# Xi-yuanWang/GLASS

Hardware: AMD Instinct MI355X
Metric: aggregated edges/sec (GLASSConv fwd+bwd) (higher is better)
Workload: dtype f32; 1 GPU; ppi_bp-shaped synthetic graph (BASELINE config[1]): N=17080, nnz=633902, hidden=64, layers=2, aggr=mean, pool=sum, z_ratio=0.95, dropout=0.5, batch=80x10 per rank, use_deg features, Adam; parallelism=subgraph-batch dp1, replicated graph, bucketed gradient all-reduce per step, step=MaxZOZ+fwd+loss+bwd+allreduce+Adam, hip_graph=True, caller=step: bench.py calls glass_amd.step.TrainStep on pre-selected batches, labels_in_head_launch=True

## Files before the change

### glass_amd/_lib.py

```python
import ctypes
import os

import torch
from ctypes import c_void_p, c_int, c_int64, c_uint64, c_float, c_double, c_char_p, POINTER

_HERE = os.path.dirname(os.path.abspath(__file__))
LIB_PATH = os.environ.get("GLASS_HIP_LIB") or os.path.join(_HERE, "libglass_hip.so")

POOL_MODES = {"sum": 0, "mean": 1, "max": 2, "size": 3}
AGGR_MODES = {"mean": 0, "sum": 1, "gcn": 2}
SEG_MODES = {"gcn": 0, "gin": 1}
ACT_NONE, ACT_ELU, ACT_RELU = 0, 1, 2
PLAN_HEADER_WORDS = 16
EMBED_NORM_MAX_ROWS = 8192
ABI_VERSION = 6


class GlassHipError(RuntimeError):
    pass


_P = c_void_p
_I = c_int64

# ... 2 lines not shown
    _fields_ = [("acc", c_void_p), ("n_rep", c_int64), ("dy", c_void_p), ("lddy", c_int64), ("x", c_void_p), ("ldx", c_int64),
                ("addend", c_void_p), ("ldadd", c_int64), ("saved", c_void_p), ("gamma", c_void_p), ("alpha", c_void_p),
                ("dgamma", c_void_p), ("dbeta", c_void_p), ("dalpha", c_void_p), ("accumulate", c_int), ("act", c_int),
                ("p_drop", c_float), ("call_id", c_uint64)]

    @property
    def ptr(self):
        return ctypes.addressof(self)


class GnSrc(ctypes.Structure):
    _fields_ = [("acc", c_void_p), ("n_src", c_int64), ("n_rep", c_int64), ("gamma", c_void_p), ("beta", c_void_p),
                ("alpha", c_void_p), ("eps", c_float)]

    @classmethod
    def of(cls, acc, n_src, n_rep, gn):
        return cls(acc.data_ptr(), n_src, n_rep, gn.weight.data_ptr(), gn.bias.data_ptr(), gn.mean_scale.data_ptr(),
                   float(gn.eps))

    @property
    def ptr(self):
        return ctypes.addressof(self)
SIGNATURES = {
    "glass_version": (c_int, []),
    "glass_last_error_string": (c_char_p, []),
    "glass_spmm_plan_build": (c_int, [_P, _I, _P, POINTER(c_int64)]),
    "glass_spmm_ws_bytes": (c_int64, [_P, _I]),
    "glass_spmm_csr_f32": (c_int, [_P, _P, _P, _P, _I, _P, _I, _I, _I, _P, _P, _P, _P]),
    "glass_adj_values_f32": (c_int, [_P, _P, _P, _I, c_int, _P, _P, _P]),
    "glass_maxzoz_i64": (c_int, [_P, _I, _P, _I, _P]),
    "glass_embed_label_f32": (c_int, [_P, _P, _I, _P, _P, _I, _P, _I, _P, _I, _I, _P]),
    "glass_mix_fwd_f32": (c_int, [_P, _I, _P, c_double, c_int, _P, _I, _I, _I, _P]),
    "glass_mix_bwd_f32": (c_int, [_P, _I, _P, _I, _P, c_double, c_int, _P, _I, _I, _I, _P]),
    "glass_graphnorm_ws_bytes": (c_int64, [_I, _I]),
    "glass_graphnorm_fwd_f32": (c_int, [_P, _I, _P, _I, _I, _I, _P, _P, _P, c_float, _P, c_int, c_float, _P, c_uint64,
                                        _P, _P]),
    "glass_graphnorm_bwd_f32": (c_int, [_P, _I, _P, _I, _P, _I, _P, _I, _I, _I, _P, _P, _P, _P, _P, _P, c_int, c_int, c_float,
                                        _P, c_uint64, _P, _P]),
    "glass_rng_advance": (c_int, [_P, _P]),
    "glass_empty_launch": (c_int, [_I, _I, _I, _I, _I, _P]),
    "glass_dropout_scales_f32": (c_int, [_P, c_uint64, c_float, _I, _I, _P, _P]),
    "glass_dual_linear_stat_rows": (c_int64, [_I]),
    "glass_copy_pair": (c_int, [_P, _P, _I, _P, _P, _I, _P]),
    "glass_graphnorm_stats_f32": (c_int, [_P, _I, _I, _I, _P, _P, _P, c_float, _P, _P, _P]),
    "glass_readout_supported": (c_int, [_I, _I, c_int]),
    "glass_readout_ws_bytes": (c_int64, [_I, _I, _I]),
    "glass_readout_train_f32": (c_int, [_P, _I, _P, _P, _P, _P, _I, _I, c_int, _P, _P, _P, c_int, _I, _P, _P, _P, _P, _P, _I,
                                        _P, _P, c_int, _P, _P, _P, c_int, _P, _I, _I, _P, _P, _P, _P, _P, c_int, _P, _P, _P]),
    "glass_readout_scatter_ws_bytes": (c_int64, [_I, _I, _I]),
    "glass_linear_wgrad_reduce_batch_f32": (c_int, [_I, _P, _P, _P, _P, _P, _P, _P, _P, _P, _P]),
    "glass_wgrad_reduce_spmm_f32": (c_int, [_I, _P, _P, _P, _P, _P, _P, _P, _P, _P, _P, _P, _P, _P, _I, _P, _I, _I, _I, _P, _P,
                                            _P, _P]),
    "glass_spmm_reduce_rows_f32": (c_int, [_P, _P, _I, _I, _P, _I, _P]),
    "glass_segment_pool_f32": (c_int, [_P, _I, _P, _I, _I, c_int, _P, _I, _P, _I, _I, _P]),
    "glass_segment_pool_bwd_f32": (c_int, [_P, _I, _P, _I, _I, c_int, _P, _P, _I, _I, _I, _P]),
    "glass_segment_pool_bwd_atomic_f32": (c_int, [_P, _I, _P, _I, _I, c_int, _P, _P, _I, _I, _I, _P]),
    "glass_segment_pool_max_bwd_exact_f32": (c_int, [_P, _I, _P, _I, _I, _P, _P, _I, _I, _I, _P, _P]),
    "glass_pair_pool_ws_bytes": (c_int64, [_I, _I]),
    "glass_segment_pool_bwd_exact_ws_bytes": (c_int64, [_I, _I, _I]),
    "glass_segment_pool_bwd_exact_f32": (c_int, [_P, _I, _P, _I, _I, c_int, _P, _I, _I, _I, _P, _P]),
    "glass_pair_pool_f32": (c_int, [_P, _I, _P, _I, c_int, _P, _I, _I, _I, _P]),
    "glass_pair_pool_bwd_f32": (c_int, [_P, _I, _P, _I, c_int, _P, _I, _I, _I, _P, _P]),
    "glass_dense_caps_query": (c_int, [_I, _P]),
    "glass_pair_head_supported": (c_int, [_I]),
    "glass_pair_head_ws_bytes": (c_int64, [_I, _I]),
    "glass_pair_head_fwd_f32": (c_int, [_P, _I, _I, _P, _I, _P, _P, _P, _P, _P, c_float, _P, c_uint64, _P, _P, _P, _P, _P, _P]),
    "glass_pair_head_bwd_f32": (c_int, [_P, _I, _I, _P, _I, _P, _P, _P, _P, c_float, _P, _P, _P, _P, c_int, _P, _P, _I, _P, _P]),
    "glass_linear_wgrad_ws_bytes": (c_int64, [_I, _I, _I]),
    "glass_linear_wgrad_f32": (c_int, [_P, _I, _P, _I, _I, _I, _I, _P, _I, _P, c_int, _P, _P]),
    "glass_dual_linear_supported": (c_int, [_I]),
    "glass_dual_linear_layout": (c_int, [_I]),
    "glass_dual_linear_fwd_f32": (c_int, [_P, _I, _P, _I, _P, _P, _P, c_double, c_int, _P, _I, _P, _I, _I, _I, _P, c_int, _P, _P,
                                          c_int, c_float, _P, c_uint64, _P, _I, _P, _I, _P]),
    "glass_dual_linear_fwd_gather_supported": (c_int, [_I]),
    "glass_step_prologue_f32": (c_int, [_P, _P, _P, _P, _P, _P, _P, _I, _P, _P, _I, _P, _P, _P, _P, c_float, _P, _P, _I, _P, _I, _P]),
    "glass_peer_allreduce_adam_f32": (c_int, [_P, _I, _P, _P, _P, _P, c_double, c_double, c_double, c_double, _P, _P, _P, _I, _P, _P]),
    "glass_peer_alloc": (c_int, [_I, _P]),
    "glass_peer_free": (c_int, [_P]),
    "glass_peer_export": (c_int, [_P, _P]),
    "glass_peer_import": (c_int, [_P, _P]),
    "glass_peer_close": (c_int, [_P]),
    "glass_step_head_f32": (c_int, [_P, _P, _P, _P, _P, _P, _P, _I, _P, _P, _I, _P, _P, _P, _P, c_float, _P, _P, _I, _P, _I,
                                    _P, _I, _I, _I, _P, _P, _P, _P, _P, _P, _I, _P]),
    "glass_graphnorm_finalize_f32": (c_int, [_P, _I, _I, _I, _I, _P, _P, _P, c_float, _P, _P]),
    "glass_graphnorm_apply_f32": (c_int, [_P, _I, _P, _I, _I, _I, _P, c_int, c_float, _P, c_uint64, _P]),
    "glass_dual_linear_dgrad_f32": (c_int, [_P, _I, _P, _I, _P, c_double, c_int, _P, _I, _P, _I, c_float, _P, c_uint64, _P, _I,
                                            _I, _I, _P, _P, _I, _P, _P, c_int, c_float, c_uint64, c_int, _P]),
    "glass_dual_linear_bwd_f32": (c_int, [_P, _I, _P, _I, _P, c_double, c_int, _P, _I, _P, _I, c_float, _P, c_uint64, _P, _I,
                                          _I, _I, _P, _P, _I, _P, _P, c_int, c_float, c_uint64, c_int, _P, _I, _P, _I, _P, _P]),
    "glass_gn_exact_supported": (c_int, [_I]),
    "glass_gn_exact_fwd_supported": (c_int, [_I]),
    "glass_gn_exact_words": (c_int64, [_I]),
    "glass_graphnorm_stats_exact_f32": (c_int, [_P, _I, _I, _I, _P, c_int, _P]),
    "glass_graphnorm_bwd_from_stats_f32": (c_int, [_P, _I, _P, _I, _P, _I, _P, _I, _I, _I, _P, _P, _P, _P, _I, _P, _P, _P,
                                                   c_int, c_int, c_float, _P, c_uint64, _P, _P]),
    "glass_embed_norm_fwd_f32": (c_int, [_P, _P, _I, _P, _P, _P, _P, c_float, _P, _P, _P, _P, _I, c_float, _P, c_uint64, _P,
                                         _I, _P, _I, _I, _P]),
    "glass_embed_norm_bwd_f32": (c_int, [_P, _P, _I, _P, _P, _P, _P, _P, c_int, _P, _P, _P, c_int, _I, _P]),
    "glass_embed_norm_bwd_adam_f32": (c_int, [_P, _P, _I, _P, _P, _P, _P, _P, c_int, _P, _P, _P, c_int, _I, _P, _P, _I, _P, _P, _P,
                                              _P, _I, _P, c_double, c_double, c_double, c_double, _P, _I, _I, _I, _I, _P]),
    "glass_dual_linear_wgrad_f32": (c_int, [_P, _I, _P, _I, _P, c_double, c_int, _P, _I, _P, _I, _I, _I, _P, _I, _P,
                                            c_int, _P, _P]),
    "glass_dense_pack_batch_f32": (c_int, [_P, _P, _P, _P, _P, _P, _P, _I, _P, _P]),
    "glass_dense_image_floats": (_I, [_I, _I, c_int]),
    "glass_dual_linear_dgrad_layout": (c_int, [_I, _I]),
    "glass_dual_linear_fwd_layout": (c_int, [_I, _I]),
    "glass_head_loss_fwd_f32": (c_int, [_P, _I, _P, _P, _P, c_int, _I, _I, _I, _P, _P, _P, _P]),
    "glass_head_linear_f32": (c_int, [_P, _I, _P, _P, _I, _I, _I, _P, _I, _P]),
    "glass_head_loss_bwd_f32": (c_int, [_P, _I, _P, _P, _P, c_int, _P, _I, _I, _I, _P, _I, _P, _P, c_int, _P]),
    "glass_batch_labels_ws_bytes": (c_int64, [_I]),
    "glass_batch_labels": (c_int, [_P, _I, _P, _P, _P, _I, _P, _P, _P, _P, _I, c_int, _P]),
    "glass_batch_labels_gather": (c_int, [_P, _I, _I, _P, _I, _P, _I, _P, _P, _P, _P, _P, _P, _I, c_int, _P]),
    "glass_comb_eff_supported": (c_int, [_I]),
    "glass_comb_eff_blocks": (c_int64, [_I, _I, _I]),
    "glass_comb_eff_fwd_blocks": (c_int64, [_I, _I, _I]),
    "glass_comb_eff_ws_bytes": (c_int64, [_I, _I, _I]),
    "glass_comb_eff_fwd_layout": (c_int, [_I]),
    "glass_comb_eff_fwd_supported": (c_int, [_I]),
    "glass_comb_eff_max_rows": (c_int64, [_I]),
    "glass_comb_eff_dgrad_layout2": (c_int, [_I]),
    "glass_comb_eff_fwd_f32": (c_int, [_P, _I, _P, _I, _P, _P, _P, c_double, _P, _I, _I, _I, _P, c_int, _P, _P, c_int, c_float, _P,
                                       c_uint64, _P, _I, _P, _P, _I, _P]),
    "glass_comb_eff_bwd_f32": (c_int, [_P, _I, _P, c_double, _P, _P, _I, _I, _I, _P, _P, _I, _P, _P, c_int, c_float, _P,
                                       c_uint64, c_int, _P, _I, _P, _I, _P, _P, _P, _I, _P, _P]),
    "glass_comb_eff_bwd_gn_src_supported": (c_int, [_I, _I]),
    "glass_adam_step_f32": (c_int, [_P, _P, _P, _P, _I, _P, c_double, c_double, c_double, c_double, _P, _P]),
    "glass_seg_extract_count": (c_int, [_P, _P, _P, _P, _P, _I, _P, _P, _I, _I, c_int, _P, _P, _P, _P]),
    "glass_seg_extract_fill": (c_int, [_P, _P, _P, _P, _P, _P, _I, _P, _P, _I, _I, c_int, _P, _P, _P, _P, _P, _P, _P, _P]),
    "glass_seg_collate": (c_int, [_P, _P, _I, _P, _P, _P, _P, _P, _P, _P, _I, _P, _I, _P, _P, _P, _P, _P, _P, _P, _P, _I,
                                  _P]),
    "glass_seg_khop_ws_bytes": (c_int64, [_I, _I]),
    "glass_seg_khop_count": (c_int, [_P, _P, _I, _P, _P, _I, _I, c_int, _P, _I, _P, _P]),
    "glass_seg_khop_fill": (c_int, [_P, _P, _I, _P, _P, _I, _I, c_int, _P, _I, _P, _P, _P]),
}

_lib = None


class DenseCaps(ctypes.Structure):
    _fields_ = [(n, ctypes.c_int32) for n in ("family", "weight_layout", "fwd_layout_trans", "fwd_layout_comb", "dgrad_layout_trans",
                                              "dgrad_layout_comb", "stat_rows", "fwd_gather", "gn_exact", "gn_exact_fwd", "comb_eff",
                                              "comb_eff_fwd", "comb_eff_fwd_layout", "comb_eff_dgrad_layout2", "pair_head", "act_codes",
                                              "product_form", "serve_width")]


_caps = {}


def dense_caps(H):
    c = _caps.get(int(H))
    if c is None:
        c = DenseCaps()
        check(load().glass_dense_caps_query(int(H), ctypes.addressof(c)), "glass_dense_caps_query")
        _caps[int(H)] = c
    return c


ACT_MASK = 0xff
DENSE_F32_PRODUCTS = 0x100


def load():
    global _lib
    if _lib is not None:
        return _lib
    if not os.path.exists(LIB_PATH):
# ... 19 lines not shown
```

### glass_amd/arena.py

```python
import torch

from .dist import FlatGradBucket


def _pairs(model):
    from .models import GLASSConv, MyGCNConv
    out = []
    for m in model.modules():
        if isinstance(m, GLASSConv):
            out.append((m, "trans", m.trans_fns[1], m.trans_fns[0]))
            out.append((m, "comb", m.comb_fns[1], m.comb_fns[0]))
        elif isinstance(m, MyGCNConv):
            out.append((m, "trans", None, m.trans_fn))
            out.append((m, "comb", None, m.comb_fn))
    return out


BIG_PARAM_ELEMS = 1 << 18

_RUNTIME_ATTRS = ("_glass_grad_bucket", "_glass_arena", "_glass_stack_prog", "_stack", "_stack_eff", "_direct_grad", "_sel_cache",
                  "_chan_cache", "_glass_train_steps", "_glass_eval_graphs", "_glass_adopted_adam")


def drop_captured_graphs(model):
# ... 83 lines not shown
            self.big_start = total
        self._exchange = None
        self.shard_optimizer = False
        self.model = model
        model._glass_grad_bucket = self
        self.params = params
        self.flat_param = torch.zeros(total, dtype=dtype, device=dev)
        self.flat = torch.zeros(total, dtype=dtype, device=dev)
        self._offsets = offsets
        drop_captured_graphs(model)
        with torch.no_grad():
            for p in params:
                o = offsets[id(p)]
                view = self.flat_param[o:o + p.numel()].view_as(p)
                view.copy_(p.data)
                p.data = view
                p.grad = self.flat[o:o + p.numel()].view_as(p)
        from .models import MyGCNConv
        for mod in model.modules():
            if isinstance(mod, (GLASSConv, MyGCNConv)):
                mod._stack = {}
                mod._stack_eff = {}
            if isinstance(mod, MyGCNConv):
                mod.z_ratio, mod.dropout = 1.0, 0.0
            if isinstance(mod, GraphNorm):
                mod._direct_grad = True
        stacks = {}
        for mod, kind, a, b in groups:
            o = stack_start[id(b)]
            n2 = 2 * b.numel()
            shape = (2 * b.shape[0], ) + tuple(b.shape[1:])
            stacks.setdefault((id(mod), kind), [mod, kind]).append(
                (self.flat_param[o:o + n2].view(shape), self.flat[o:o + n2].view(shape)))
        self._packs = []
        from . import _lib
        for (_, kind), (mod, _k, *views) in stacks.items():
            if len(views) == 2:
                (W, dW), (b, db) = views
                O, K = W.shape
                from . import ops
                if ops.dual_linear_supported(O // 2) and _lib.load().glass_dual_linear_layout(O // 2) == 2:
                    mod._stack[kind] = (W, b, dW, db, W, W)
                elif O % 64 == 0 and K % 64 == 0 and ops.dual_linear_supported(O // 2):
                    tiled = _lib.load().glass_dual_linear_layout(O // 2) == 1
                    dlay = int(_lib.load().glass_dual_linear_dgrad_layout(O // 2, K))
                    flay = int(_lib.load().glass_dual_linear_fwd_layout(O // 2, K))
                    Wimg = torch.empty(int(_lib.load().glass_dense_image_floats(O, K, 0 | (flay << 1))), dtype=W.dtype, device=W.device)
                    WTimg = torch.empty(int(_lib.load().glass_dense_image_floats(K, O, 1 | (dlay << 1))), dtype=W.dtype, device=W.device)
                    self._packs.append((W, Wimg, O, K, 0 | (flay << 1), mod))
                    self._packs.append((W, WTimg, K, O, 1 | (dlay << 1), mod))
                    mod._stack[kind] = (W, b, dW, db, Wimg, WTimg)
                    if kind == "comb" and K == O and _lib.load().glass_comb_eff_supported(O // 2):
                        lay2 = int(_lib.load().glass_comb_eff_dgrad_layout2(O // 2))
                        We = torch.empty_like(Wimg)
                        WTe = torch.empty(WTimg.numel() * (2 if lay2 else 1), dtype=W.dtype, device=W.device)
                        self._packs.append((W, We, O, K, 0 | (int(_lib.load().glass_comb_eff_fwd_layout(O // 2)) << 1), mod))
                        self._packs.append((W, WTe, K, O, 1 | (7 << 1), mod))
                        if lay2:
                            self._packs.append((W, WTe[WTimg.numel():], K, O, 1 | (lay2 << 1), mod))
                        mod._stack_eff = {"comb": (We, WTe)}
                    elif kind == "comb" and K == O and _lib.load().glass_comb_eff_fwd_supported(O // 2):
                        We = torch.empty(W.numel(), dtype=W.dtype, device=W.device)
                        self._packs.append((W, We, O, K, 0 | (int(_lib.load().glass_comb_eff_fwd_layout(O // 2)) << 1), mod))
                        mod._stack_eff = {"comb": (We, None)}
                else:
                    mod._stack[kind] = (W, b, dW, db)
        import numpy as np
        self._pack_args = (np.array([w.data_ptr() for w, *_ in self._packs], dtype=np.uint64),
                           np.array([p[1].data_ptr() for p in self._packs], dtype=np.uint64),
                           np.array([p[1].numel() for p in self._packs], dtype=np.int64),
                           np.array([p[2] for p in self._packs], dtype=np.int64),
                           np.array([p[3] for p in self._packs], dtype=np.int64),
                           np.array([p[4] for p in self._packs], dtype=np.int32),
                           np.zeros(len(self._packs), dtype=np.float32), len(self._packs))
        from .models import EmbZGConv, EmbGConv
        for mod in model.modules():
            if isinstance(mod, (EmbZGConv, EmbGConv)):
                mod._glass_arena = self
        self.refresh_transposes()

    def refresh_transposes(self, rng_state=None, table=None, zero=None, head=None):
        src, dst, cap, nt, kt, tr, zr, k = self._pack_args
        from . import _lib, ops
        for i, p in enumerate(self._packs):
            zr[i] = float(getattr(p[5], "z_ratio", 0.0))
        if k == 0 and rng_state is not None and table is None and zero is None and head is None:
            ops.rng_advance(rng_state.device)
        for i in range(0, max(k, 1), 16):
            n = min(16, k - i)
            rng = rng_state.data_ptr() if (rng_state is not None and i == 0) else 0
            st = torch.cuda.current_stream().cuda_stream
            if (table is not None or zero is not None or head is not None) and i == 0:
                zargs = (0, 0) if zero is None else (zero.data_ptr(), zero.numel())
                if table is not None:
                    W, V, rowptr, gn, saved, tab = table
                    targs = (W.data_ptr(), V, rowptr.data_ptr(), gn.weight.data_ptr(), gn.bias.data_ptr(), gn.mean_scale.data_ptr(),
                             float(gn.eps), saved.data_ptr(), 0 if tab is None else tab.data_ptr(), W.shape[1])
                else:
                    targs = (0, 0, 0, 0, 0, 0, 0.0, 0, 0, 0)
                if head is not None:
                    rc = _lib.load().glass_step_head_f32(src[i:].ctypes.data, dst[i:].ctypes.data, cap[i:].ctypes.data, nt[i:].ctypes.data,
                                                         kt[i:].ctypes.data, tr[i:].ctypes.data, zr[i:].ctypes.data, max(n, 0), rng,
                                                         *targs, *zargs, *head.head_args(), st)
                    _lib.check(rc, "glass_step_head_f32")
                    head.loaded = True
                else:
                    rc = _lib.load().glass_step_prologue_f32(src[i:].ctypes.data, dst[i:].ctypes.data, cap[i:].ctypes.data, nt[i:].ctypes.data,
                                                             kt[i:].ctypes.data, tr[i:].ctypes.data, zr[i:].ctypes.data, max(n, 0), rng,
                                                             *targs, *zargs, st)
                    _lib.check(rc, "glass_step_prologue_f32")
            elif n > 0:
                rc = _lib.load().glass_dense_pack_batch_f32(src[i:].ctypes.data, dst[i:].ctypes.data, cap[i:].ctypes.data, nt[i:].ctypes.data,
                                                            kt[i:].ctypes.data, tr[i:].ctypes.data, zr[i:].ctypes.data, n, rng, st)
                _lib.check(rc, "glass_dense_pack_batch_f32")
            else:
                continue
            if rng_state is not None and i == 0:
                ops.note_rng_advance(rng_state.device)

    def offset_of(self, param):
        return self._offsets.get(id(param))

    def attached(self):
        base_p, base_g = self.flat_param.untyped_storage().data_ptr(), self.flat.untyped_storage().data_ptr()
        return all(p.data.untyped_storage().data_ptr() == base_p and p.grad is not None
                   and p.grad.untyped_storage().data_ptr() == base_g for p in self.params)

    def reattach(self):
        base_p = self.flat_param.untyped_storage().data_ptr()
        base_g = self.flat.untyped_storage().data_ptr()
        if any(p.data.untyped_storage().data_ptr() != base_p for p in self.params):
            drop_captured_graphs(self.model)
        with torch.no_grad():
            for p in self.params:
                o = self._offsets[id(p)]
                if p.data.untyped_storage().data_ptr() != base_p:
                    view = self.flat_param[o:o + p.numel()].view_as(p)
                    view.copy_(p.data)
                    p.data = view
                if p.grad is None or p.grad.untyped_storage().data_ptr() != base_g:
                    p.grad = self.flat[o:o + p.numel()].view_as(p)

    @property
    def exchange(self):
        from . import dist as gdist
        if self._exchange is None and gdist.is_distributed():
            self._exchange = gdist.GradExchange(self.flat, self.flat_param, self.big_start)
        return self._exchange

    def sharded(self):
        ex = self.exchange
        return self.shard_optimizer and ex is not None and ex.has_big

    def adopt_grad_storage(self, flat):
        if flat.numel() != self.flat.numel() or flat.dtype != self.flat.dtype or flat.device != self.flat.device:
            raise ValueError("adopt_grad_storage: the new buffer must match the gradient arena")
        drop_captured_graphs(self.model)
        for mod in self.model.modules():
            mod.__dict__.pop("_glass_stack_prog", None)
        self.flat = flat
        self._exchange = None
        with torch.no_grad():
            for p in self.params:
                o = self._offsets[id(p)]
                p.grad = self.flat[o:o + p.numel()].view_as(p)
        for mod in self.model.modules():
            st = getattr(mod, "_stack", None)
            if isinstance(st, dict):
                for kind, tup in list(st.items()):
                    W, b, dW, db = tup[:4]
                    oW = W.data_ptr() - self.flat_param.data_ptr()
                    ob = b.data_ptr() - self.flat_param.data_ptr()
                    ndW = self.flat[oW // 4:oW // 4 + W.numel()].view_as(W)
                    ndb = self.flat[ob // 4:ob // 4 + b.numel()].view_as(b)
                    st[kind] = (W, b, ndW, ndb) + tuple(tup[4:])

    def all_reduce_mean(self):
        if getattr(self, "_peer", None) is not None:
            return
        ex = self.exchange
        if ex is None:
            return
        if ex.has_big and not self.shard_optimizer:
            FlatGradBucket.all_reduce_mean(self)
            return
        ex.reduce_small()
        ex.reduce_big()

    def zero(self):
        if not self.attached():
            raise RuntimeError("ParamArena detached (model.to()/zero_grad(set_to_none=True) after flattening?)")
        self.flat.zero_()
```

### glass_amd/csrc/dense.hip

```cpp
#include "common.h"
#include "dense_common.h"
#include "labels_body.h"
#include "split_mma.h"
#include "wgrad_common.h"
#include "emb_table.h"

#ifndef GLASS_WGRAD_STAGED
#define GLASS_WGRAD_STAGED 0
#endif

#include <stdlib.h>

namespace glass {

#ifndef GLASS_COMB_BWD_V2
#define GLASS_COMB_BWD_V2 0
#endif
#ifndef GLASS_SL_STAGED2
#define GLASS_SL_STAGED2 1
#endif
#ifndef GLASS_COMB_DGRAD_V2
#define GLASS_COMB_DGRAD_V2 1
#endif
#ifndef GLASS_TRANS_DGRAD_V2
#define GLASS_TRANS_DGRAD_V2 1
#endif
#ifndef GLASS_TRANS_WGRAD_STAGED2
#define GLASS_TRANS_WGRAD_STAGED2 1
#endif
#ifndef GLASS_TRANS_FWD_V2
#define GLASS_TRANS_FWD_V2 1
#endif
#ifndef GLASS_COMB_FWD_V2
#define GLASS_COMB_FWD_V2 1
#endif
#ifndef GLASS_FUSED_WGRAD_STAGES
#define GLASS_FUSED_WGRAD_STAGES 2
#endif
#if !GLASS_LAB && (GLASS_WGRAD_STAGED || GLASS_COMB_BWD_V2 || !GLASS_SL_STAGED2 || !GLASS_COMB_DGRAD_V2 || !GLASS_TRANS_DGRAD_V2 ||       \
                   !GLASS_TRANS_WGRAD_STAGED2 || !GLASS_TRANS_FWD_V2 || !GLASS_COMB_FWD_V2)
#error "the variant switches above select laboratory forms whose kernels live in tools/lab/: build with -DGLASS_LAB=1 (tools/build_trace.sh)"
#endif
#ifdef GLASS_DENSE_TRACE
__device__ unsigned long long* g_dense_trace;
__device__ int g_dense_trace_sel;
#endif


typedef float f32x4 __attribute__((ext_vector_type(4)));

constexpr int kKC = 16;

__device__ __forceinline__ void load16(float (&dst)[kKC], const float* p, bool ok) {
#pragma unroll
    for (int v = 0; v < kKC / 4; ++v) {
        float4 t = ok ? *reinterpret_cast<const float4*>(p + 4 * v) : make_float4(0.f, 0.f, 0.f, 0.f);
        dst[4 * v] = t.x; dst[4 * v + 1] = t.y; dst[4 * v + 2] = t.z; dst[4 * v + 3] = t.w;
    }
}

__device__ __forceinline__ int tile_col(int t, int j) { return 64 * (t >> 2) + 4 * j + (t & 3); }

template <int NT, int THREADS>
struct WStage {
    static constexpr int NTILES = NT / 16;
    static constexpr int kVecs = NTILES * 4 * 64;
    static constexpr int kPerThread = kVecs / THREADS;
    static constexpr int kHalf = kPerThread / 2;
    static_assert(kPerThread % 2 == 0, "staging is held as two half arrays");
    float4 ra[kHalf], rb[kHalf];
    __device__ __forceinline__ void fetch(const float* __restrict__ Wimg, int kc) {
        const float4* src = reinterpret_cast<const float4*>(Wimg) + (int64_t)kc * kVecs;
#pragma unroll
        for (int n = 0; n < kHalf; ++n) {
            ra[n] = src[threadIdx.x + THREADS * n];
            rb[n] = src[threadIdx.x + THREADS * (kHalf + n)];
        }
    }
    __device__ __forceinline__ void commit(float4* __restrict__ image) const {
#pragma unroll
        for (int n = 0; n < kHalf; ++n) {
            image[threadIdx.x + THREADS * n] = ra[n];
            image[threadIdx.x + THREADS * (kHalf + n)] = rb[n];
        }
    }
};

template <int NTILES, int HALF>
// ... 2530 lines not shown
__global__ __launch_bounds__(kBlock, 2) void comb_bwd_eff_kernel(DgradEffArgs A, int n_dgrad_blocks, WgradSL sl, float zr,
                                                                float* __restrict__ part_w, float* __restrict__ part_b) {
    extern __shared__ float4 lds_w[];
    const int n_wg_blocks = (int)gridDim.x - n_dgrad_blocks;
    const int b = (int)blockIdx.x < n_wg_blocks ? n_dgrad_blocks + (int)blockIdx.x : (int)blockIdx.x - n_wg_blocks;
    if (b == 0 && threadIdx.x == 0) {
        float* header = part_b + (int64_t)(sl.n_s + sl.n_l) * kSLOut;
        header[0] = 2.f;
        header[1] = zr;
        header[2] = GLASS_SL_STAGED2 ? 1.f : 0.f;
    }
    if (b < n_dgrad_blocks) {
        D_STAMP(3, 0);
        if (GLASS_COMB_DGRAD_V2) {
            DgradEffArgs A2 = A;
            A2.WT = A.WT + 2 * (2 * H * H);
            if (A.gs.partial && A.gs.drop.p > 0.f)
                comb_dgrad2_body<H, true, SP>(A2, b, reinterpret_cast<float*>(lds_w));
            else
                comb_dgrad2_body<H, false, SP>(A2, b, reinterpret_cast<float*>(lds_w));
        } else {
            comb_dgrad_eff_body<H, 4>(A.dsrc, A.ldd, A.mask, A.WT, A.rng_state, A.out, A.ldo, A.N, A.gs, A.lab, b, lds_w);
        }
        D_STAMP(3, 4);
        return;
    }
    D_STAMP(3, 5);
    float* lds = reinterpret_cast<float*>(lds_w);
    if (GLASS_SL_STAGED2) {
        if constexpr (SP)
            wgrad_sl_staged2s_body(sl, A.N, b - n_dgrad_blocks, part_w, part_b, lds);
        else
            wgrad_sl_staged2_body(sl, A.N, b - n_dgrad_blocks, part_w, part_b, lds);
        D_STAMP(3, 6);
        return;
    }
    if (GLASS_WGRAD_STAGED && sl.rows_per_slab <= kStageRows)
        wgrad_sl_staged_body(sl, A.N, b - n_dgrad_blocks, part_w, part_b, lds, lds + 2 * kTile);
    else
        wgrad_sl_body<GLASS_FUSED_WGRAD_STAGES>(sl, A.N, b - n_dgrad_blocks, part_w, part_b, lds, lds + 2 * kTile);
    D_STAMP(3, 6);
}

struct PackJob {
    const float* src;
    float* dst;
    int NT, KT, transposed, layout;
    float zr;
    int cut;
};
constexpr int kMaxPackJobs = 16;
struct PackBatch {
    PackJob job[kMaxPackJobs];
};

__device__ __forceinline__ float4 pack_fetch(const PackJob& j, int n, int k) {
    if (!j.transposed) return *reinterpret_cast<const float4*>(j.src + (int64_t)n * j.KT + k);
    return make_float4(j.src[(int64_t)k * j.NT + n], j.src[(int64_t)(k + 1) * j.NT + n], j.src[(int64_t)(k + 2) * j.NT + n],
                       j.src[(int64_t)(k + 3) * j.NT + n]);
}

__device__ __forceinline__ void pack_cut_put(float* cut, int tile, int nl, int q, const float4& v) {
    const Split4 s = split4(v);
    uint2* p = reinterpret_cast<uint2*>(cut) + (((size_t)tile * 6 + (q >> 1)) * 256 + nl) * 2 + (q & 1);
    p[0] = s.hi;
    p[1024] = s.mid;
    p[2048] = s.lo;
}

struct TableJob {
    const float* W;
    int V, H;
    const int32_t* rowptr;
    const float *gamma, *beta, *alpha;
    float eps;
    float *saved, *table;
};

struct ZeroJob {
    long long* p;
    int64_t n;
};

__device__ __forceinline__ void pack_batch_body(const PackBatch& batch, uint64_t* rng_state, const TableJob& tab, int n_jobs,
                                                const ZeroJob& zero, int rows) {
    if (rng_state && blockIdx.x == 0 && blockIdx.y == 0 && threadIdx.x == 0) rng_state[1] += 1;
    if (zero.p) {
        const int64_t nthreads = (int64_t)gridDim.x * rows * kBlock;
        for (int64_t k = ((int64_t)blockIdx.y * gridDim.x + blockIdx.x) * kBlock + threadIdx.x; k < zero.n; k += nthreads) zero.p[k] = 0;
    }
    if ((int)blockIdx.y >= n_jobs) {
        __shared__ double tab_lds[kBlock * 2];
        __shared__ float tab_coef[2 * kTabCols];
        if (tab.W && (int)blockIdx.x < (tab.H + kTabCols - 1) / kTabCols)
            emb_table_fwd_block(blockIdx.x, tab.W, tab.V, tab.H, tab.rowptr, tab.gamma, tab.beta, tab.alpha, tab.eps, tab.saved,
                                tab.table, tab_lds, tab_coef);
        return;
    }
    const PackJob j = batch.job[blockIdx.y];
    const int total = j.NT * j.KT / 4;
    if (j.layout == kLayoutWave16 || j.layout == kLayoutWave16Cols) {
        const int KQ = j.KT / 4, NTILES = j.NT / 16;
        const bool cols = j.layout == kLayoutWave16Cols;
        for (int l = blockIdx.x * kBlock + threadIdx.x; l < total; l += gridDim.x * kBlock) {
            const int lane = l & 63, v = (l >> 6) & 3, t = (l >> 8) % NTILES, kc = (l >> 8) / NTILES;
            const int jj = lane & 15, q = lane >> 4;
            const int n = cols ? 64 * (t >> 2) + 16 * (t & 3) + jj : tile_col(t, jj);
            reinterpret_cast<float4*>(j.dst)[l] = pack_fetch(j, n, q * KQ + kc * kKC + 4 * v);
        }
        return;
    }
    if (j.layout == kLayoutWave16EffFwd || j.layout == kLayoutWave16EffDgrad || j.layout == kLayoutWave16EffFwdCols ||
        j.layout == kLayoutWave16EffDgradCols) {
        const bool fwd = j.layout == kLayoutWave16EffFwd || j.layout == kLayoutWave16EffFwdCols;
        const bool cols = j.layout == kLayoutWave16EffFwdCols || j.layout == kLayoutWave16EffDgradCols;
        const int NTe = fwd ? j.NT / 2 : j.NT, KTe = fwd ? j.KT : j.KT / 2;
        const int KQ = KTe / 4, NTILES = NTe / 16, per = NTe * KTe / 4;
        const float zr = j.zr, omz = 1.f - j.zr;
        for (int l = blockIdx.x * kBlock + threadIdx.x; l < 2 * per; l += gridDim.x * kBlock) {
            const int img = l >= per, ll = img ? l - per : l;
            const int lane = ll & 63, v = (ll >> 6) & 3, t = (ll >> 8) % NTILES, kc = (ll >> 8) / NTILES;
            const int jj = lane & 15, q = lane >> 4;
            const int n = cols ? 64 * (t >> 2) + 16 * (t & 3) + jj : tile_col(t, jj), k = q * KQ + kc * kKC + 4 * v;
            const float4 a = pack_fetch(j, n, k);
            const float4 b = fwd ? pack_fetch(j, j.NT / 2 + n, k) : pack_fetch(j, n, j.KT / 2 + k);
            const float c1 = img ? zr : omz, c0 = img ? omz : zr;
            reinterpret_cast<float4*>(j.dst)[l] = make_float4(c1 * a.x + c0 * b.x, c1 * a.y + c0 * b.y, c1 * a.z + c0 * b.z,
                                                              c1 * a.w + c0 * b.w);
        }
        return;
    }
    if (j.layout == kLayoutTiledSplit) {
        const int NKS = j.KT / 32;
        for (int l = blockIdx.x * kBlock + threadIdx.x; l < total; l += gridDim.x * kBlock) {
            const int nl = l & 255, q = (l >> 8) & 3, ks = l >> 10;
            const int v = tiled_col(kLayoutTiledPlain, 0, nl, 0);
            if (ks < NKS) {
                const float4 e = pack_fetch(j, v % j.NT, (v / j.NT) * (j.KT / 2) + 16 * ks + 4 * q);
                reinterpret_cast<float4*>(j.dst)[l] = e;
                if (j.cut) pack_cut_put(j.dst + 4 * (size_t)total, ks, nl, q, e);
            }
        }
        return;
    }
    const int NKS = j.KT / 16, H = j.NT / 2;
    const int lay = j.layout == kLayoutTiledPlainEff ? kLayoutTiledPlain : j.layout == kLayoutTiledPairedEff ? kLayoutTiledPaired : j.layout;
    const bool has_app = j.layout == kLayoutTiledPlainEff || j.layout == kLayoutTiledPairedEff;
    float* cut = j.dst + 4 * (size_t)total + (has_app ? 2 * (size_t)total : 0);
    for (int l = blockIdx.x * kBlock + threadIdx.x; l < total; l += gridDim.x * kBlock) {
        const int nl = l & 255, q = (l >> 8) & 3, tile = l >> 10;
        const int ct = tile / NKS, ks = tile % NKS;
        const float4 e = pack_fetch(j, tiled_col(lay, ct, nl, H), 16 * ks + 4 * q);
        reinterpret_cast<float4*>(j.dst)[l] = e;
        if (j.cut) pack_cut_put(cut, tile, nl, q, e);
    }
    if (j.layout == kLayoutTiledPairedEff) {
        float4* app = reinterpret_cast<float4*>(j.dst) + total;
        const float zr = j.zr, omz = 1.f - j.zr;
        for (int l = blockIdx.x * kBlock + threadIdx.x; l < total / 2; l += gridDim.x * kBlock) {
            const int nl = l & 255, q = (l >> 8) & 3, tile = l >> 10;
            const int ct = tile / NKS, ks = tile % NKS;
            const int n = tiled_col(kLayoutTiledPlain, ct, nl, H), k = 16 * ks + 4 * q;
            const float4 a = pack_fetch(j, n, k), b = pack_fetch(j, H + n, k);
            const float4 e = make_float4(omz * a.x + zr * b.x, omz * a.y + zr * b.y, omz * a.z + zr * b.z, omz * a.w + zr * b.w);
            app[l] = e;
            if (j.cut) pack_cut_put(cut, total / 1024 + tile, nl, q, e);
        }
        return;
    }
    if (j.layout != kLayoutTiledPlainEff) return;
    const int NKS2 = NKS / 2;
    float4* app = reinterpret_cast<float4*>(j.dst) + total;
    const float zr = j.zr, omz = 1.f - j.zr;
    for (int l = blockIdx.x * kBlock + threadIdx.x; l < total / 2; l += gridDim.x * kBlock) {
        const int nl = l & 255, q = (l >> 8) & 3, tile = l >> 10;
        const int ct = tile / NKS2, ks = tile % NKS2;
        const int n = tiled_col(kLayoutTiledPlain, ct, nl, H), k = 16 * ks + 4 * q;
        const float4 a = pack_fetch(j, n, k), b = pack_fetch(j, n, j.KT / 2 + k);
        const float4 e = make_float4(omz * a.x + zr * b.x, omz * a.y + zr * b.y, omz * a.z + zr * b.z, omz * a.w + zr * b.w);
        app[l] = e;
        if (j.cut) pack_cut_put(cut, total / 1024 + tile, nl, q, e);
    }
}

__global__ __launch_bounds__(kBlock) void pack_batch_kernel(PackBatch batch, uint64_t* rng_state, TableJob tab, int n_jobs,
                                                            ZeroJob zero) {
    pack_batch_body(batch, rng_state, tab, n_jobs, zero, (int)gridDim.y);
}

struct LabelJob {
    glass_batch_cursor* cur;
    int n_idx, smax, y_row_words;
    int64_t* pos_dst;
    uint32_t* y_dst;
    uint8_t* mask;
    int32_t *lab_rows, *lab_count, *owner;
    int64_t N;
};

__global__ __launch_bounds__(kLabThreads) void step_head_kernel(PackBatch batch, uint64_t* rng_state, TableJob tab, int n_jobs,
                                                                ZeroJob zero, int rows, LabelJob lj) {
    if ((int)blockIdx.y < rows) {
        if (threadIdx.x >= kBlock) return;
        pack_batch_body(batch, rng_state, tab, n_jobs, zero, rows);
        return;
    }
    if (blockIdx.x != 0) return;
    const int64_t n_b = lj.cur->n_batches, c = lj.cur->cursor;
    const int64_t b = c < 0 ? 0 : (lj.cur->wrap ? c % n_b : (c >= n_b ? n_b - 1 : c));
    const BatchSrc src{lj.cur->pos_all, reinterpret_cast<const uint32_t*>(lj.cur->y_all), lj.cur->idx + b * lj.n_idx, lj.smax,
                       lj.y_row_words > 0 ? lj.y_row_words : 1, lj.cur->n_all};
    batch_labels_body<true>(src, lj.n_idx * lj.smax, lj.pos_dst, lj.y_dst, (int64_t)lj.n_idx * lj.y_row_words, lj.mask, lj.lab_rows,
                            lj.lab_count, lj.owner, lj.N, 1);
    if (threadIdx.x == 0) lj.cur->cursor = c + 1;
}

}

using namespace glass;

template <typename K>
static void allow_lds(K kernel, size_t bytes) {
    if (bytes > 64 * 1024) (void)hipFuncSetAttribute((const void*)kernel, hipFuncAttributeMaxDynamicSharedMemorySize, (int)bytes);
}

static bool wave16_shape_ok(int64_t H) { return H == 64; }
static bool h64_split_products() { return tiled_split_products() && lab_knob("GLASS_H64_SPLIT", 1) != 0; }
static int fwd_wave_groups(bool comb) {
    const int forced = lab_knob("GLASS_FWD_WG", 0);
    if (forced == 1 || forced == 2) return forced;
    return comb ? 1 : 2;
}
static bool tiled_here(int64_t H) { return tiled_shape_ok(H) && !wave16_shape_ok(H); }
static bool dense_shape_ok(int64_t H) { return wave16_shape_ok(H) || tiled_shape_ok(H) || narrow_shape_ok(H); }
static size_t lds_bytes(int64_t NT, int n_pass) {
    const size_t image = (size_t)NT * 256;
    return n_pass > 1 ? 2 * image : image;
}

#ifdef GLASS_DENSE_TRACE
extern "C" int glass_dense_trace_set(unsigned long long* p, int sel) {
    int rc = (int)hipMemcpyToSymbol(HIP_SYMBOL(g_dense_trace), &p, sizeof(p));
    return rc ? rc : (int)hipMemcpyToSymbol(HIP_SYMBOL(g_dense_trace_sel), &sel, sizeof(sel));
}
#endif
extern "C" int glass_gn_exact_supported(int64_t H) { return wave16_shape_ok(H) ? 1 : 0; }
extern "C" int glass_gn_exact_fwd_supported(int64_t H) { return (wave16_shape_ok(H) || (GLASS_COMB_FWD_V2 && H == 128)) ? 1 : 0; }
static bool rep_ok(int64_t n_rep) { return n_rep == 2 || n_rep == 4 || n_rep == 8 || n_rep == 16; }
static bool make_exact_src(const glass_gn_src* g, const float* saved, GnExactSrc& out) {
    out = GnExactSrc{nullptr, 1, kAccRep, nullptr, nullptr, nullptr, 0.f, nullptr};
    if (!g) return true;
    if (!g->acc || g->n_src != 1 || !rep_ok(g->n_rep) || !g->gamma || !g->beta || !g->alpha || !saved) return false;
    out = GnExactSrc{reinterpret_cast<const long long*>(g->acc), 1, (int)g->n_rep, g->gamma, g->beta, g->alpha, g->eps,
                     const_cast<float*>(saved)};
    return true;
}
extern "C" int64_t glass_gn_exact_words(int64_t C) { return gn_acc_words(C); }

extern "C" int glass_dual_linear_supported(int64_t H) { return dense_shape_ok(H) ? 1 : 0; }

extern "C" int glass_pair_head_supported(int64_t hidden);
extern "C" int glass_dense_caps_query(int64_t H, glass_dense_caps* out) {
    GLASS_REQUIRE(H > 0 && out, "dense_caps: H > 0 and a record to fill");
    glass_dense_caps c{};
    c.family = narrow_shape_ok(H) ? 1 : wave16_shape_ok(H) ? 2 : tiled_here(H) ? 3 : 0;
    if (c.family) {
        c.weight_layout = glass_dual_linear_layout(H);
        c.fwd_layout_trans = glass_dual_linear_fwd_layout(H, H);
        c.fwd_layout_comb = glass_dual_linear_fwd_layout(H, 2 * H);
        c.dgrad_layout_trans = glass_dual_linear_dgrad_layout(H, H);
        c.dgrad_layout_comb = glass_dual_linear_dgrad_layout(H, 2 * H);
        c.stat_rows = (int32_t)glass_dual_linear_stat_rows(H);
        c.fwd_gather = glass_dual_linear_fwd_gather_supported(H);
        c.act_codes = (1 << GLASS_ACT_ELU) | (1 << GLASS_ACT_RELU);
        c.product_form = (c.family == 3 || (c.family == 2 && lab_knob("GLASS_H64_SPLIT", 1) != 0)) ? 1 : 0;
    }
    c.serve_width = c.family ? (int32_t)H : (H <= 64 ? 64 : H <= 128 ? 128 : H <= 256 ? 256 : H <= 512 ? 512 : 0);
    c.gn_exact = glass_gn_exact_supported(H);
    c.gn_exact_fwd = glass_gn_exact_fwd_supported(H);
    c.comb_eff = glass_comb_eff_supported(H);
    c.comb_eff_fwd = glass_comb_eff_fwd_supported(H);
    c.comb_eff_fwd_layout = c.comb_eff_fwd ? glass_comb_eff_fwd_layout(H) : 0;
    c.comb_eff_dgrad_layout2 = c.comb_eff ? glass_comb_eff_dgrad_layout2(H) : 0;
    c.pair_head = glass_pair_head_supported(H);
    *out = c;
    return 0;
}
extern "C" int glass_dual_linear_fwd_gather_supported(int64_t H) { return (wave16_shape_ok(H) || narrow_shape_ok(H) || tiled_here(H)) ? 1 : 0; }

extern "C" int glass_dual_linear_layout(int64_t H) { return narrow_shape_ok(H) ? 2 : tiled_here(H) ? 1 : 0; }

extern "C" int glass_dual_linear_fwd_layout(int64_t H, int64_t K) {
    if (GLASS_TRANS_FWD_V2 && (wave16_shape_ok(H) || H == 128) && K == H) return kLayoutWave16Cols;
    if (!tiled_here(H)) return kLayoutWave16;
    return tiled_eff_fwd_shape(H, K) ? kLayoutTiledPairedEff : kLayoutTiledPaired;
}
extern "C" int glass_dual_linear_dgrad_layout(int64_t H, int64_t n_out) {
// ... 496 lines not shown
        const glass_gn_bwd_src& g = *dsrc_gn;
        if (!glass_comb_eff_bwd_gn_src_supported(n_nodes, H) || !X) {
            set_error("comb_eff_bwd: dsrc_gn is served by the staged fused launch only (hidden 64, small graphs, with the weight gradient)");
            return GLASS_E_UNSUPPORTED;
        }
        GLASS_REQUIRE(g.acc && rep_ok(g.n_rep) && g.dy && g.x && g.saved && g.gamma && g.alpha && g.lddy >= H && g.lddy % 4 == 0 &&
                          g.ldx >= H && g.ldx % 4 == 0 && aligned16(g.dy) && aligned16(g.x) && aligned16(g.saved) &&
                          (!g.addend || (g.ldadd >= H && g.ldadd % 4 == 0 && aligned16(g.addend))) && g.p_drop >= 0.f && g.p_drop < 1.f &&
                          (g.p_drop == 0.f || rng_state) && act_code_ok(g.act) &&
                          n_nodes * std::max(std::max(g.lddy, g.ldx), g.addend ? g.ldadd : (int64_t)0) * 4 < (1ll << 31),
                      "comb_eff_bwd: bad dsrc_gn");
        gsrc = GnBwdSrc{reinterpret_cast<const long long*>(g.acc), (int)g.n_rep, g.dy, g.lddy, g.x, g.ldx, g.addend, g.ldadd, g.saved,
                        g.gamma, g.alpha, g.dgamma, g.dbeta, g.dalpha, g.accumulate, g.act, make_drop(g.p_drop, g.call_id, H)};
        if (!dsrc) {
            dsrc = g.dy;
            ldd = g.lddy;
        }
    }
    if (H != 64) {
        set_error("comb_eff_bwd: hidden size %lld not supported (64)", (long long)H);
        return GLASS_E_UNSUPPORTED;
    }
    GLASS_REQUIRE(ldd >= H && ldd % 4 == 0 && aligned16(dsrc) && aligned16(WTimg_eff) && ldo >= 2 * H && ldo % 4 == 0 &&
                      aligned16(out),
                  "comb_eff_bwd: operands must be 16-B aligned with ld %% 4 == 0");
    GLASS_REQUIRE(!gn_partial || (gn_x && gn_saved && gn_alpha && gn_ldx >= H && gn_ldx % 4 == 0 && aligned16(gn_x) &&
                                  aligned16(gn_saved) && aligned16(gn_alpha) && gn_p_drop >= 0.f && gn_p_drop < 1.f &&
                                  (gn_p_drop == 0.f || rng_state) && act_code_ok(gn_act)),
                  "comb_eff_bwd: bad GraphNorm statistics arguments");
    GLASS_REQUIRE(!gn_exact || (gn_partial && rep_ok(gn_exact)), "comb_eff_bwd: gn_exact = replicas of the accumulators (2, 4, 8, 16)");
    hipStream_t st = (hipStream_t)stream;
    const int n_main = (int)ceil_div(n_nodes, 64);
    const unsigned n_dg = (unsigned)(n_main + ceil_div(lab_cap, 64));
    const float zr = (float)z_ratio;
    const GnBwdStats gs{gn_partial, gn_exact, gn_x, gn_ldx, gn_saved, gn_alpha, gn_act, make_drop(gn_partial ? gn_p_drop : 0.f, gn_call_id, H)};
    const DgradEffArgs dargs{dsrc, ldd, mask, WTimg_eff, rng_state, out, ldo, n_nodes, gs, LabRows{lab_rows, lab_count, n_main, (int)lab_cap}, gsrc};
    const size_t lds_dg = lds_bytes(2 * H, 1);
    if (!X) {
        hipLaunchKernelGGL((comb_dgrad_eff_kernel<64>), dim3(n_dg), dim3(kBlock), lds_dg, st, dargs);
        return launch_status("glass_comb_eff_bwd_f32 (dgrad)");
    }
    GLASS_REQUIRE(X2 && ws && ldx >= H && ldx % 4 == 0 && aligned16(X) && ldx2 >= H && ldx2 % 4 == 0 && aligned16(X2) &&
                      aligned16(ws),
                  "comb_eff_bwd: the pair's inputs must be 16-B aligned with ld %% 4 == 0");
    const WgradSLGeom g = wgrad_sl_geom(n_nodes, lab_cap);
    float* part_w = (float*)ws;
    float* part_b = part_w + g.part_w_floats;
    const WgradSL sl{dsrc, ldd, X, ldx, X2, ldx2, lab_rows, lab_count, g.n_s, g.rows_per_slab, g.n_l, gsrc, rng_state};
    if (n_nodes > kFusedBwdMaxRows) {
        hipLaunchKernelGGL((comb_dgrad_eff_kernel<64>), dim3(n_dg), dim3(kBlock), lds_dg, st, dargs);
        launch_wgrad_sl(sl, n_nodes, zr, part_w, part_b, st);
        return launch_status("glass_comb_eff_bwd_f32 (two launches)");
    }
#if GLASS_LAB && GLASS_COMB_BWD_V2
#include "../../tools/lab/dispatch_comb_bwd_v2.inc"
#endif
    if (GLASS_COMB_DGRAD_V2) {
        GLASS_REQUIRE(gn_act == GLASS_ACT_NONE, "comb_eff_bwd: the GraphNorm in front of the comb pair has no activation");
        const int64_t ld_max = std::max(std::max(std::max(ldd, ldo), gn_partial ? gn_ldx : (int64_t)0), std::max(ldx, ldx2));
        GLASS_REQUIRE(n_nodes * ld_max * 4 < (1ll << 31), "comb_eff_bwd: n_nodes * ld * 4 must stay below 2^31 (32-bit buffer offsets)");
    }
    const size_t lds_wg = (size_t)(2 * kTile + 8 * kSLOut) * sizeof(float);
    static_assert(kCombDgrad2Lds <= (size_t)(2 * kTile + 8 * kSLOut) * sizeof(float), "the staged data gradient fits the fused launch's LDS");
    const size_t lds_fused = lds_dg > lds_wg ? lds_dg : lds_wg;
    if (h64_split_products() && GLASS_COMB_DGRAD_V2 && GLASS_SL_STAGED2 && g.rows_per_slab % 32 == 0) {
        const size_t lds_sp = std::max(kCombDgrad2SplitLds, kStg2sLdsBytes);
        allow_lds(comb_bwd_eff_kernel<64, true>, lds_sp);
        hipLaunchKernelGGL((comb_bwd_eff_kernel<64, true>), dim3(n_dg + (unsigned)(g.n_s + g.n_l)), dim3(kBlock), lds_sp, st, dargs,
                           (int)n_dg, sl, zr, part_w, part_b);
        return launch_status("glass_comb_eff_bwd_f32");
    }
    allow_lds(comb_bwd_eff_kernel<64>, lds_fused);
    hipLaunchKernelGGL((comb_bwd_eff_kernel<64>), dim3(n_dg + (unsigned)(g.n_s + g.n_l)), dim3(kBlock), lds_fused, st, dargs,
                       (int)n_dg, sl, zr, part_w, part_b);
    return launch_status("glass_comb_eff_bwd_f32");
}

extern "C" int64_t glass_comb_eff_ws_bytes(int64_t n_nodes, int64_t H, int64_t lab_cap) {
    if (H != 64 || n_nodes <= 0 || lab_cap < 0) return GLASS_E_ARG;
    const WgradSLGeom g = wgrad_sl_geom(n_nodes, lab_cap);
    return (g.part_w_floats + g.part_b_floats) * (int64_t)sizeof(float);
}

static int pack_launch(const float* const* src, float* const* dst, const int64_t* dst_floats, const int64_t* NT, const int64_t* KT,
                       const int32_t* transposed, const float* z_ratio, int64_t n_jobs, uint64_t* rng_state,
                       const TableJob& tab, void* stream, const char* what, ZeroJob zero = ZeroJob{nullptr, 0},
                       const LabelJob* lj = nullptr) {
    GLASS_REQUIRE(n_jobs >= 0 && n_jobs <= kMaxPackJobs && (n_jobs == 0 || (src && dst && dst_floats && NT && KT && transposed)),
                  "%s: bad arguments (at most %d matrices per call)", what, kMaxPackJobs);
    PackBatch b;
    for (int k = 0; k < kMaxPackJobs; ++k) b.job[k] = PackJob{nullptr, nullptr, 0, 0, 0, 0, 0.f, 0};
    for (int k = 0; k < n_jobs; ++k) {
        GLASS_REQUIRE(src[k] && dst[k] && NT[k] > 0 && NT[k] % 64 == 0 && KT[k] > 0 && KT[k] % 64 == 0 && aligned16(src[k]) &&
                          aligned16(dst[k]),
                      "%s: job %d needs NT, KT multiples of 64 and 16-B aligned buffers", what, k);
        const int layout = transposed[k] >> 1;
        GLASS_REQUIRE(dst_floats[k] >= glass_dense_image_floats(NT[k], KT[k], transposed[k]),
                      "%s: job %d: dst holds %lld floats, the image of this layout needs %lld (glass_dense_image_floats)", what, k,
                      (long long)dst_floats[k], (long long)glass_dense_image_floats(NT[k], KT[k], transposed[k]));
        GLASS_REQUIRE(layout == kLayoutWave16 ||
                          (layout == kLayoutWave16Cols && ((NT[k] == 128 && KT[k] == 64 && !(transposed[k] & 1)) ||
                                                           (NT[k] == 256 && KT[k] == 128 && !(transposed[k] & 1)) ||
                                                           (NT[k] == 64 && KT[k] == 128 && (transposed[k] & 1)) ||
                                                           (NT[k] == 128 && KT[k] == 256 && (transposed[k] & 1)))) ||
                          ((layout == kLayoutTiledPaired || layout == kLayoutTiledPlain) && NT[k] % 256 == 0) ||
                          (layout == kLayoutTiledSplit && NT[k] == 128 && KT[k] == 256 && (transposed[k] & 1)) ||
                          (layout == kLayoutTiledPlainEff && NT[k] % 256 == 0 && KT[k] % 32 == 0 && (transposed[k] & 1) && z_ratio) ||
                          (layout == kLayoutTiledPairedEff && NT[k] % 512 == 0 && !(transposed[k] & 1) && z_ratio) ||
                          ((layout == kLayoutWave16EffFwd || layout == kLayoutWave16EffFwdCols) && NT[k] % 128 == 0 &&
                           !(transposed[k] & 1) && z_ratio) ||
                          ((layout == kLayoutWave16EffDgrad || layout == kLayoutWave16EffDgradCols) && KT[k] % 128 == 0 &&
                           (transposed[k] & 1) && z_ratio),
                      "%s: job %d: unknown layout %d, NT not a multiple of 256 for a tiled layout, or a split "
                      "layout that is not the transposed 128 x 256 operand", what, k, layout);
        const bool tiled_layout = layout == kLayoutTiledPaired || layout == kLayoutTiledPlain || layout == kLayoutTiledSplit ||
                                  layout == kLayoutTiledPlainEff || layout == kLayoutTiledPairedEff;
        b.job[k] = PackJob{src[k], dst[k], (int)NT[k], (int)KT[k], transposed[k] & 1, layout, z_ratio ? z_ratio[k] : 0.f,
                           tiled_layout ? 1 : 0};
    }
    unsigned gx = 32;
    if (tab.W && (unsigned)ceil_div(tab.H, kTabCols) > gx) gx = (unsigned)ceil_div(tab.H, kTabCols);
    unsigned gy = (unsigned)n_jobs + (tab.W ? 1u : 0u);
    if (gy == 0) gy = 1;
    if (lj)
        hipLaunchKernelGGL(step_head_kernel, dim3(gx, gy + 1), dim3(kLabThreads), 0, (hipStream_t)stream, b, rng_state, tab, (int)n_jobs,
                           zero, (int)gy, *lj);
    else
        hipLaunchKernelGGL(pack_batch_kernel, dim3(gx, gy), dim3(kBlock), 0, (hipStream_t)stream, b, rng_state, tab, (int)n_jobs, zero);
    return launch_status(what);
}

extern "C" int64_t glass_dense_image_floats(int64_t NT, int64_t KT, int32_t flags) {
    if (NT <= 0 || KT <= 0) return GLASS_E_ARG;
    const int layout = flags >> 1;
    int64_t base = NT * KT;
    if (layout == kLayoutTiledPlainEff || layout == kLayoutTiledPairedEff) base += base / 2;
    const bool tiled_layout = layout == kLayoutTiledPaired || layout == kLayoutTiledPlain || layout == kLayoutTiledSplit ||
                              layout == kLayoutTiledPlainEff || layout == kLayoutTiledPairedEff;
    return tiled_layout ? base + base * 3 / 2 : base;
}

extern "C" int glass_dense_pack_batch_f32(const float* const* src, float* const* dst, const int64_t* dst_floats,
                                          const int64_t* NT, const int64_t* KT, const int32_t* transposed,
                                          const float* z_ratio, int64_t n_jobs, uint64_t* rng_state, void* stream) {
    GLASS_REQUIRE(src && dst && dst_floats && NT && KT && transposed && n_jobs >= 0 && n_jobs <= kMaxPackJobs,
                  "dense_pack_batch: bad arguments (at most %d matrices per call)", kMaxPackJobs);
    if (n_jobs == 0) return rng_state ? glass_rng_advance(rng_state, stream) : 0;
    return pack_launch(src, dst, dst_floats, NT, KT, transposed, z_ratio, n_jobs, rng_state, TableJob{}, stream, "glass_dense_pack_batch_f32");
}

extern "C" int glass_step_prologue_f32(const float* const* src, float* const* dst, const int64_t* dst_floats,
                                       const int64_t* NT, const int64_t* KT, const int32_t* transposed, const float* z_ratio, int64_t n_jobs, uint64_t* rng_state,
                                       const float* W, int64_t V, const int32_t* class_rowptr, const float* gamma,
                                       const float* beta, const float* alpha, float eps, float* saved, float* table,
                                       int64_t H, int64_t* zero_words, int64_t n_zero_words, void* stream) {
    GLASS_REQUIRE(!W || (class_rowptr && gamma && beta && alpha && saved && H > 0 && V > 0 && V <= GLASS_EMBED_NORM_MAX_ROWS),
                  "step_prologue: bad embedding-table arguments (at most %d rows)", GLASS_EMBED_NORM_MAX_ROWS);
    GLASS_REQUIRE(n_zero_words >= 0 && (n_zero_words == 0 || zero_words), "step_prologue: bad zero-fill arguments");
    TableJob tab{};
    if (W) tab = TableJob{W, (int)V, (int)H, class_rowptr, gamma, beta, alpha, eps, saved, table};
    return pack_launch(src, dst, dst_floats, NT, KT, transposed, z_ratio, n_jobs, rng_state, tab, stream, "glass_step_prologue_f32",
                       ZeroJob{n_zero_words > 0 ? (long long*)zero_words : nullptr, n_zero_words});
}

extern "C" int glass_step_head_f32(const float* const* src, float* const* dst, const int64_t* dst_floats, const int64_t* NT,
                                   const int64_t* KT, const int32_t* transposed, const float* z_ratio, int64_t n_jobs,
                                   uint64_t* rng_state, const float* W, int64_t V, const int32_t* class_rowptr, const float* gamma,
                                   const float* beta, const float* alpha, float eps, float* saved, float* table, int64_t H,
                                   int64_t* zero_words, int64_t n_zero_words, glass_batch_cursor* cur, int64_t n_idx,
                                   int64_t smax, int64_t y_row_bytes, int64_t* pos_dst, void* y_dst, uint8_t* mask,
                                   int32_t* lab_rows, int32_t* lab_count, void* ws, int64_t n_nodes, void* stream) {
    GLASS_REQUIRE(!W || (class_rowptr && gamma && beta && alpha && saved && H > 0 && V > 0 && V <= GLASS_EMBED_NORM_MAX_ROWS),
                  "step_head: bad embedding-table arguments (at most %d rows)", GLASS_EMBED_NORM_MAX_ROWS);
    GLASS_REQUIRE(n_zero_words >= 0 && (n_zero_words == 0 || zero_words), "step_head: bad zero-fill arguments");
    GLASS_REQUIRE(cur && pos_dst && mask && lab_rows && lab_count && ws, "step_head: null pointer");
    GLASS_REQUIRE(smax > 0 && n_idx > 0 && n_idx * smax < (1ll << 30) && n_nodes > 0 && n_nodes < (1ll << 31) &&
                      (reinterpret_cast<uintptr_t>(cur) & 7u) == 0,
                  "step_head: bad sizes");
    GLASS_REQUIRE(y_row_bytes == 0 || (y_dst && y_row_bytes > 0 && y_row_bytes % 4 == 0 && y_row_bytes < (1ll << 30) &&
                                       (reinterpret_cast<uintptr_t>(y_dst) & 3u) == 0),
                  "step_head: the target rows have 4-byte granularity");
    TableJob tab{};
    if (W) tab = TableJob{W, (int)V, (int)H, class_rowptr, gamma, beta, alpha, eps, saved, table};
    const LabelJob lj{cur, (int)n_idx, (int)smax, (int)(y_row_bytes / 4), pos_dst, (uint32_t*)y_dst, mask, lab_rows, lab_count,
                      (int32_t*)ws, n_nodes};
    return pack_launch(src, dst, dst_floats, NT, KT, transposed, z_ratio, n_jobs, rng_state, tab, stream, "glass_step_head_f32",
                       ZeroJob{n_zero_words > 0 ? (long long*)zero_words : nullptr, n_zero_words}, &lj);
}
```

### glass_amd/csrc/embnorm.hip

```cpp
#include "common.h"
#include "emb_table.h"
#include "gn_math.h"

namespace glass {

__global__ __launch_bounds__(kBlock) void emb_table_fwd_kernel(const float* __restrict__ W, int V, int H,
                                                               const int32_t* __restrict__ rowptr,
                                                               const float* __restrict__ gamma,
                                                               const float* __restrict__ beta,
                                                               const float* __restrict__ alpha, float eps,
                                                               float* __restrict__ saved, float* __restrict__ table,
                                                               uint8_t* __restrict__ mask_fill, int fill_value,
                                                               int64_t n_nodes) {
    __shared__ double lds[kBlock * 2];
    __shared__ float coef[2 * kTabCols];
    if (mask_fill)
        for (int64_t n = (int64_t)blockIdx.x * kBlock + threadIdx.x; n < n_nodes; n += (int64_t)gridDim.x * kBlock)
            mask_fill[n] = (uint8_t)fill_value;
    if ((int)blockIdx.x >= (H + kTabCols - 1) / kTabCols) return;
    emb_table_fwd_block(blockIdx.x, W, V, H, rowptr, gamma, beta, alpha, eps, saved, table, lds, coef);
}

__global__ __launch_bounds__(kBlock) void emb_table_bwd_kernel(const float* __restrict__ G, const float* __restrict__ W,
                                                               int V, int H, const int32_t* __restrict__ rowptr,
                                                               const float* __restrict__ gamma,
                                                               const float* __restrict__ alpha,
                                                               const float* __restrict__ saved, float* __restrict__ dW,
                                                               int accumulate_w, float* __restrict__ dgamma,
                                                               float* __restrict__ dbeta, float* __restrict__ dalpha,
                                                               int accumulate) {
    __shared__ double lds[kBlock * 2];
    __shared__ float coef[3 * kTabCols];
    const int tc = threadIdx.x & (kTabCols - 1), tr = threadIdx.x / kTabCols;
    const int c = blockIdx.x * kTabCols + tc;
    const bool ok = c < H;
    double s1 = 0.0, s2 = 0.0;
    if (ok) {
        const float mu = saved[c], rstd = saved[H + c], al = alpha[c];
        for (int v = tr; v < V; v += kTabSlots) {
            const float g = G[(int64_t)v * H + c];
            const float xhat = (W[(int64_t)v * H + c] - al * mu) * rstd;
            s1 += (double)g;
            s2 += (double)g * (double)xhat;
        }
    }
    slot_reduce(s1, s2, lds, tc, tr);
    if (tr == 0 && ok) {
        float A, Bx, K, da;
        gn_bwd_coeffs(s1, s2, (double)rowptr[V], gamma[c], alpha[c], saved[c], saved[H + c], A, Bx, K, da);
        if (dgamma) dgamma[c] = (accumulate ? dgamma[c] : 0.f) + (float)s2;
        if (dbeta) dbeta[c] = (accumulate ? dbeta[c] : 0.f) + (float)s1;
        if (dalpha) dalpha[c] = (accumulate ? dalpha[c] : 0.f) + da;
        coef[tc] = A;
        coef[kTabCols + tc] = Bx;
        coef[2 * kTabCols + tc] = K;
    }
    __syncthreads();
    if (!ok) return;
    const float A = coef[tc], Bx = coef[kTabCols + tc], K = coef[2 * kTabCols + tc];
    for (int v = tr; v < V; v += kTabSlots) {
        const int64_t o = (int64_t)v * H + c;
        const float cn = (float)(rowptr[v + 1] - rowptr[v]);
        const float d = fmaf(A, G[o], cn * fmaf(Bx, W[o], K));
        dW[o] = accumulate_w ? dW[o] + d : d;
    }
}

struct TailAdam {
    float* p;
    float* g;
    float *m, *v;
    int64_t n;
    const float* lr;
    float beta1, beta2, eps, weight_decay;
    int64_t* step;
    int64_t off_W, off_gamma, off_beta, off_alpha;
};

__global__ __launch_bounds__(kBlock) void emb_tail_kernel(float* __restrict__ G, const float* W, int V, int H,
                                                          const int32_t* __restrict__ rowptr,
                                                          const float* gamma, const float* alpha,
                                                          const float* __restrict__ saved, float* dW,
                                                          int accumulate_w, float* __restrict__ dgamma,
                                                          float* __restrict__ dbeta, float* __restrict__ dalpha,
                                                          int accumulate, const float* __restrict__ partials,
                                                          const int32_t* __restrict__ rrows, int n_reduce, TailAdam ad,
                                                          int n_tab) {
    __shared__ double lds[kBlock * 2];
    __shared__ float coef[3 * kTabCols];
    int64_t step_now = 0;
    AdamCoef ac{};
    if (ad.p) {
        step_now = ad.step[0] + 1;
        ac = adam_coef(step_now, ad.lr[0], ad.beta1, ad.beta2, ad.eps, ad.weight_decay);
    }
    if ((int)blockIdx.x >= n_tab) {
        const int64_t nb = (int64_t)gridDim.x - n_tab;
        const int64_t tab_lo = ad.off_W, tab_hi = ad.off_W + (int64_t)V * H;
        for (int64_t k = ((int64_t)blockIdx.x - n_tab) * kBlock + threadIdx.x; k < ad.n; k += nb * kBlock) {
            if ((k >= tab_lo && k < tab_hi) || (k >= ad.off_gamma && k < ad.off_gamma + H) ||
                (k >= ad.off_beta && k < ad.off_beta + H) || (k >= ad.off_alpha && k < ad.off_alpha + H))
                continue;
            adam_update(ac, ad.p, ad.g[k], ad.m, ad.v, k);
        }
        adam_ticket(ad.step, step_now);
        return;
    }
    const int tc = threadIdx.x & (kTabCols - 1), tr = threadIdx.x / kTabCols;
    const int c = blockIdx.x * kTabCols + tc;
    const bool ok = c < H;
    constexpr int kOwn = 4;
    const bool small = V <= kOwn * kTabSlots;
    float w_own[kOwn], cn_own[kOwn], m_own[kOwn], v_own[kOwn];
    if (small) {
#pragma unroll
        for (int k = 0; k < kOwn; ++k) {
            const int v = tr + kTabSlots * k;
            const bool live = ok && v < V;
            const int64_t o = (int64_t)(live ? v : 0) * H + (ok ? c : 0);
            w_own[k] = live ? W[o] : 0.f;
            cn_own[k] = live ? (float)(rowptr[v + 1] - rowptr[v]) : 0.f;
            m_own[k] = (live && ad.p) ? ad.m[ad.off_W + o] : 0.f;
            v_own[k] = (live && ad.p) ? ad.v[ad.off_W + o] : 0.f;
        }
    }
    if (ok)
        for (int rr = tr; rr < n_reduce; rr += kTabSlots) {
            const int row = rrows[3 * rr], first = rrows[3 * rr + 1], n = rrows[3 * rr + 2];
            float sum = 0.f;
            for (int k = 0; k < n; ++k) sum += partials[(int64_t)(first + k) * H + c];
            G[(int64_t)row * H + c] = sum;
        }
    if (n_reduce > 0) __syncthreads();
    double s1 = 0.0, s2 = 0.0;
    float g_own[kOwn];
    if (ok && small) {
        const float mu = saved[c], rstd = saved[H + c], al = alpha[c];
#pragma unroll
        for (int k = 0; k < kOwn; ++k) {
            const int v = tr + kTabSlots * k;
            g_own[k] = v < V ? G[(int64_t)v * H + c] : 0.f;
        }
#pragma unroll
        for (int k = 0; k < kOwn; ++k) {
            if (tr + kTabSlots * k >= V) continue;
            const float xhat = (w_own[k] - al * mu) * rstd;
            s1 += (double)g_own[k];
            s2 += (double)g_own[k] * (double)xhat;
        }
    } else if (ok) {
        const float mu = saved[c], rstd = saved[H + c], al = alpha[c];
        for (int v = tr; v < V; v += kTabSlots) {
            const float g = G[(int64_t)v * H + c];
            const float xhat = (W[(int64_t)v * H + c] - al * mu) * rstd;
            s1 += (double)g;
            s2 += (double)g * (double)xhat;
        }
    }
    slot_reduce(s1, s2, lds, tc, tr);
    if (tr == 0 && ok) {
        float A, Bx, K, da;
        gn_bwd_coeffs(s1, s2, (double)rowptr[V], gamma[c], alpha[c], saved[c], saved[H + c], A, Bx, K, da);
        const float g_gamma = (accumulate ? dgamma[c] : 0.f) + (float)s2;
        const float g_beta = (accumulate ? dbeta[c] : 0.f) + (float)s1;
        const float g_alpha = (accumulate ? dalpha[c] : 0.f) + da;
        dgamma[c] = g_gamma;
        dbeta[c] = g_beta;
        dalpha[c] = g_alpha;
        coef[tc] = A;
        coef[kTabCols + tc] = Bx;
        coef[2 * kTabCols + tc] = K;
        if (ad.p) {
            adam_update(ac, ad.p, g_gamma, ad.m, ad.v, ad.off_gamma + c);
            adam_update(ac, ad.p, g_beta, ad.m, ad.v, ad.off_beta + c);
            adam_update(ac, ad.p, g_alpha, ad.m, ad.v, ad.off_alpha + c);
        }
    }
    __syncthreads();
    if (ok && small) {
        const float A = coef[tc], Bx = coef[kTabCols + tc], K = coef[2 * kTabCols + tc];
#pragma unroll
        for (int k = 0; k < kOwn; ++k) {
            const int v = tr + kTabSlots * k;
            if (v >= V) continue;
            const int64_t o = (int64_t)v * H + c;
            float d = fmaf(A, g_own[k], cn_own[k] * fmaf(Bx, w_own[k], K));
            if (accumulate_w) d += dW[o];
            dW[o] = d;
            if (ad.p) {
                float pk = w_own[k];
                adam_element(ac, pk, d, m_own[k], v_own[k]);
                ad.m[ad.off_W + o] = m_own[k];
                ad.v[ad.off_W + o] = v_own[k];
                ad.p[ad.off_W + o] = pk;
            }
        }
    } else if (ok) {
        const float A = coef[tc], Bx = coef[kTabCols + tc], K = coef[2 * kTabCols + tc];
        for (int v = tr; v < V; v += kTabSlots) {
            const int64_t o = (int64_t)v * H + c;
            const float cn = (float)(rowptr[v + 1] - rowptr[v]);
            float d = fmaf(A, G[o], cn * fmaf(Bx, W[o], K));
            if (accumulate_w) d += dW[o];
            dW[o] = d;
            if (ad.p) adam_update(ac, ad.p, d, ad.m, ad.v, ad.off_W + o);
        }
    }
    if (ad.p) adam_ticket(ad.step, step_now);
}

template <int VW> struct Vg;
template <> struct Vg<4> {
    float a[4];
    __device__ __forceinline__ void load(const float* p) {
        float4 v = *reinterpret_cast<const float4*>(p);
        a[0] = v.x; a[1] = v.y; a[2] = v.z; a[3] = v.w;
    }
    __device__ __forceinline__ void store(float* p) const {
        *reinterpret_cast<float4*>(p) = make_float4(a[0], a[1], a[2], a[3]);
    }
};
template <> struct Vg<1> {
    float a[1];
    __device__ __forceinline__ void load(const float* p) { a[0] = *p; }
    __device__ __forceinline__ void store(float* p) const { *p = a[0]; }
};

constexpr int kUnrollG = 4;

template <int VW>
__global__ __launch_bounds__(kBlock) void embed_gather_kernel(const int64_t* __restrict__ x,
                                                              const float* __restrict__ table, int64_t V,
                                                              const int64_t* __restrict__ z,
                                                              const int64_t* __restrict__ pos, int64_t n_pos,
                                                              float* __restrict__ out, int64_t ldo,
                                                              uint8_t* __restrict__ mask, int64_t N, int H,
                                                              int tc_log2, Drop drop,
                                                              const uint64_t* __restrict__ rng_state) {
    const int TC = 1 << tc_log2, rpb = kBlock >> tc_log2;
    const int tc = threadIdx.x & (TC - 1), tr = threadIdx.x >> tc_log2;
    const int c0 = (blockIdx.y * TC + tc) * VW;
    if (blockIdx.y == 0) {
        if (z) {
            for (int64_t n = (int64_t)blockIdx.x * kBlock + threadIdx.x; n < N; n += (int64_t)gridDim.x * kBlock)
                mask[n] = z[n] > 0 ? 1 : 0;
        } else if (pos) {
            for (int64_t i = (int64_t)blockIdx.x * kBlock + threadIdx.x; i < n_pos; i += (int64_t)gridDim.x * kBlock) {
                const int64_t p = pos[i];
                if (p >= 0 && p < N) mask[p] = 1;
            }
        }
    }
    if (c0 >= H) return;
    if (drop.p > 0.f) {
        drop.seed = rng_state[0];
        drop.step = rng_state[1];
    }
    const int64_t stride = (int64_t)gridDim.x * rpb;
    for (int64_t r = (int64_t)blockIdx.x * rpb + tr; r < N; r += stride * kUnrollG) {
        Vg<VW> v[kUnrollG];
#pragma unroll
        for (int u = 0; u < kUnrollG; ++u) {
            const int64_t rr = r + u * stride;
#pragma unroll
            for (int k = 0; k < VW; ++k) v[u].a[k] = 0.f;
            if (rr < N) {
                const int64_t idx = x[rr];
                if (idx >= 0 && idx < V) v[u].load(table + idx * H + c0);
            }
        }
#pragma unroll
        for (int u = 0; u < kUnrollG; ++u) {
            const int64_t rr = r + u * stride;
            if (rr >= N) continue;
            if (drop.p > 0.f) {
                float ds[VW];
                drop_scales<VW>(drop, rr, c0, ds);
#pragma unroll
                for (int k = 0; k < VW; ++k) v[u].a[k] *= ds[k];
            }
            v[u].store(out + rr * ldo + c0);
        }
    }
}

}

using namespace glass;

extern "C" int glass_embed_norm_fwd_f32(const int64_t* x, const float* W, int64_t V, const int32_t* class_rowptr,
// ... 85 lines not shown
```

### glass_amd/stack.py

```python
import os

import numpy as np
import torch

from . import _lib, ops
from .ops import ACT_ELU, ACT_NONE, ACT_RELU, _stream

USE_EMBED_TABLE = os.environ.get("GLASS_EMBED_TABLE", "1") != "0"
USE_READOUT = os.environ.get("GLASS_READOUT", "1") != "0"


def _check(rc, what):
    _lib.check(rc, what)


USE_GN_EXACT = os.environ.get("GLASS_GN_EXACT", "1") != "0"
USE_READOUT_TWO = os.environ.get("GLASS_READOUT_TWO", "1") != "0"
USE_GN_BWD_IN_COMB = os.environ.get("GLASS_GN_BWD_IN_COMB", "1") != "0"
USE_GN_EXACT_FWD = os.environ.get("GLASS_GN_EXACT_FWD", "1") != "0"
GN_EXACT_MAX_ROWS = 1 << 18
GN_EXACT_FWD_ONLY_MAX_ROWS = 1 << 14
GN_EXACT_READOUT_MAX_ROWS = 1 << 16
USE_FUSED_TAIL = os.environ.get("GLASS_FUSED_TAIL", "1") != "0"
USE_GATHER_IN_TRANS = os.environ.get("GLASS_GATHER_IN_TRANS", "1") != "0"
USE_COMB_EFF = os.environ.get("GLASS_COMB_EFF", "1") != "0"


_PROLOGUE_DONE = False


class prologue_done:
    def __init__(self, on=True):
        self.on = bool(on)

    def __enter__(self):
        global _PROLOGUE_DONE
        self.prev, _PROLOGUE_DONE = _PROLOGUE_DONE, (self.on or _PROLOGUE_DONE)

    def __exit__(self, *exc):
        global _PROLOGUE_DONE
        _PROLOGUE_DONE = self.prev


class BatchLabels:
    def __init__(self, n_nodes, cap, device):
        self.n, self.cap = int(n_nodes), int(cap)
        self.mask = torch.zeros(self.n, dtype=torch.uint8, device=device)
        self.rows = torch.zeros(max(self.cap, 1), dtype=torch.int32, device=device)
        self.count = torch.zeros(4, dtype=torch.int32, device=device)
        self.ws = torch.full((self.n,), 2**31 - 1, dtype=torch.int32, device=device)
        self.loaded = False
        self.cursor = None
        self._epoch = None
        self.in_head = False

    def set_epoch(self, pos_all, y_all, idx_batches, pos_dst, y_dst, wrap=False):
        n_all, smax = pos_all.shape
        n_b, n_idx = idx_batches.shape
        if n_idx * smax != self.cap:
            raise ValueError(f"BatchLabels: batches of {n_idx * smax} entries, capacity {self.cap}")
        yrb = 0 if y_all is None else y_all.element_size() * (y_all.numel() // max(y_all.shape[0], 1))
        if self.cursor is None:
            self.cursor = torch.zeros(8, dtype=torch.int64, device=self.mask.device)
        desc = torch.tensor([pos_all.data_ptr(), 0 if y_all is None else y_all.data_ptr(), idx_batches.data_ptr(), n_all, n_b, 0, 1 if wrap else 0, 0],
                            dtype=torch.int64)
        self.cursor.copy_(desc)
        self._epoch = (pos_all, y_all, idx_batches, pos_dst, y_dst, int(n_idx), int(smax), int(yrb))

    def rewind(self):
        if self.cursor is not None:
            self.cursor[5:6].zero_()

    def head_args(self):
        _pos_all, y_all, _idx, pos_dst, y_dst, n_idx, smax, yrb = self._epoch
        return (self.cursor.data_ptr(), n_idx, smax, yrb, pos_dst.data_ptr(), 0 if y_all is None else y_dst.data_ptr(),
                self.mask.data_ptr(), self.rows.data_ptr(), self.count.data_ptr(), self.ws.data_ptr(), self.n)

    def head_signature(self):
        return None if self._epoch is None else self._epoch[5:]

    def load(self, pos_src, pos_dst=None, y_src=None, y_dst=None):
        if pos_src.numel() != self.cap:
            raise ValueError(f"BatchLabels: batch of {pos_src.numel()} entries, capacity {self.cap}")
        yb = 0 if y_src is None else y_src.numel() * y_src.element_size()
        incremental = 1 if pos_dst is not None else 0
        rc = _lib.load().glass_batch_labels(pos_src.data_ptr(), pos_src.numel(), 0 if pos_dst is None else pos_dst.data_ptr(),
                                            0 if y_src is None else y_src.data_ptr(), 0 if y_dst is None else y_dst.data_ptr(),
                                            yb, self.mask.data_ptr(), self.rows.data_ptr(), self.count.data_ptr(),
                                            self.ws.data_ptr(), self.n, incremental, _stream())
        _check(rc, "glass_batch_labels")
        self.loaded = True

    def load_gather(self, pos_all, y_all, idx, pos_dst, y_dst):
        n_all, smax = pos_all.shape
        if idx.numel() * smax != self.cap:
            raise ValueError(f"BatchLabels: batch of {idx.numel() * smax} entries, capacity {self.cap}")
        yrb = 0 if y_all is None else y_all.element_size() * (y_all.numel() // max(y_all.shape[0], 1))
        rc = _lib.load().glass_batch_labels_gather(pos_all.data_ptr(), n_all, smax, 0 if y_all is None else y_all.data_ptr(), yrb,
                                                   idx.data_ptr(), idx.numel(), pos_dst.data_ptr(),
                                                   0 if y_all is None else y_dst.data_ptr(), self.mask.data_ptr(),
                                                   self.rows.data_ptr(), self.count.data_ptr(), self.ws.data_ptr(), self.n, 1,
                                                   _stream())
        _check(rc, "glass_batch_labels_gather")
        self.loaded = True


def _comb_eff_ld(emb, H):
    return max(4 * H, H * len(emb.convs) if emb.jk else H)
# ... 311 lines not shown
        mods = [emb.emb_gn] + [c.gn for c in emb.convs] + list(emb.gns)
        return all(getattr(m, "_direct_grad", False) and m.weight.grad is not None for m in mods) and \
            emb.input_emb.weight.grad is not None

    def forward(self, x_flat, z, edge_index, edge_weight, keep, readout=None, acc=1, labels=None, snapshot_rng=False):
        dev = x_flat.device
        with ops.rng_scope(dev, None):
            return self._forward(x_flat, z, edge_index, edge_weight, keep, readout, acc, labels, snapshot_rng)

    def _forward(self, x_flat, z, edge_index, edge_weight, keep, readout, acc, labels, snapshot_rng):
        from .models import buildAdj
        emb, lib = self.emb, _lib.load()
        dev = x_flat.device
        n = x_flat.shape[0]
        W = emb.input_emb.weight
        V, H = W.shape
        L = len(emb.convs)
        train = emb.training
        p = float(emb.dropout) if train else 0.0
        f32 = dict(dtype=torch.float32, device=dev)
        advance = train and (p > 0 or any(c.dropout > 0 for c in emb.convs))
        from .models import _act_code
        act = _act_code(emb.activation)
        st = {"n": n, "H": H, "L": L, "p": p, "x_flat": x_flat, "acc": int(acc), "rng_epoch": ops.rng_epoch(dev), "act": act,
              "stat_rows": int(lib.glass_dual_linear_stat_rows(H))}
        unl = not hasattr(emb, "emb_gn")
        st["unlabeled"] = unl
        if unl:
            labels = emb.__dict__.get("_glass_no_labels")
            if labels is None or labels.n != n or labels.mask.device != dev:
                labels = emb.__dict__["_glass_no_labels"] = BatchLabels(n, 1, dev)
                labels.loaded = True
        if isinstance(z, tuple) and labels is None and train:
            labels = BatchLabels(n, z[1].numel(), dev)
            labels.load(z[1])
        if labels is not None:
            zp, pp, npos = 0, 0, -1
            mask = labels.mask
        elif isinstance(z, tuple):
            zp, pp, npos = 0, z[1].data_ptr(), z[1].numel()
            mask = torch.empty(n, dtype=torch.uint8, device=dev)
        else:
            zp, pp, npos = (0 if z is None else z.data_ptr()), 0, 0
            mask = torch.empty(n, dtype=torch.uint8, device=dev)
        st["labels"] = labels
        h = torch.empty((n, H), **f32)
        st["mask"] = mask
        gn0 = None if unl else emb.emb_gn
        use_table = (V <= _lib.EMBED_NORM_MAX_ROWS and USE_EMBED_TABLE) or unl
        first_gn = None
        acc_all = acc_bwd = acc_fwd = acc_ro = None
        exact_all = USE_GN_EXACT and bool(lib.glass_gn_exact_supported(H)) and n <= GN_EXACT_MAX_ROWS
        exact_fwd_only = (not exact_all and USE_GN_EXACT and n <= GN_EXACT_FWD_ONLY_MAX_ROWS and
                          bool(lib.glass_gn_exact_fwd_supported(H)) and L == 1 and
                          all(_comb_eff_fwd_ok(conv, labels, H, _comb_eff_ld(emb, H)) for conv in emb.convs))
        if exact_all or exact_fwd_only:
            n_bwd = 2 * L - 1 if (keep and exact_all) else 0
            n_fwd = 2 * L if ((readout is not None or unl) and USE_GN_EXACT_FWD) else 0
            w_h = int(lib.glass_gn_exact_words(H))
            w_ro = int(lib.glass_gn_exact_words(H * L if emb.jk else H)) if (readout is not None and keep and USE_READOUT_TWO) else 0
            if n_bwd + n_fwd:
                acc_all = torch.empty((n_bwd + n_fwd) * w_h + w_ro, dtype=torch.int64, device=dev)
                blocks = acc_all[:(n_bwd + n_fwd) * w_h].view(n_bwd + n_fwd, w_h)
                acc_bwd = blocks[:n_bwd] if n_bwd else None
                acc_fwd = blocks[n_bwd:] if n_fwd else None
                acc_ro = acc_all[(n_bwd + n_fwd) * w_h:] if w_ro else None
        elif (USE_GN_EXACT and USE_READOUT_TWO and readout is not None and keep and labels is not None and H % 4 == 0 and
              (H * L if emb.jk else H) <= 128 and n <= GN_EXACT_READOUT_MAX_ROWS):
            acc_all = acc_ro = torch.empty(int(lib.glass_gn_exact_words(H * L if emb.jk else H)), dtype=torch.int64, device=dev)
        st["gn_exact"] = acc_bwd
        st["gn_exact_readout"] = acc_ro
        head = labels if (labels is not None and getattr(labels, "in_head", False) and train) else None
        if unl:
            sel = emb._selection(x_flat)
            ident = emb.__dict__.get("_glass_ident_saved")
            if ident is None or ident.device != dev:
                ident = emb.__dict__["_glass_ident_saved"] = torch.cat([torch.zeros(H, **f32), torch.ones(2 * H, **f32), torch.zeros(H, **f32)])
            emb._glass_arena.refresh_transposes(ops.rng_state(dev) if advance else None, zero=acc_all, head=head)
            st["emb_table"], st["emb_saved"] = sel, ident
            first_gn = (ident, ACT_NONE, p, 1)
        elif use_table and labels is not None and USE_GATHER_IN_TRANS and lib.glass_dual_linear_fwd_gather_supported(H):
            sel = emb._selection(x_flat)
            saved = torch.empty(4 * H, **f32)
            emb._glass_arena.refresh_transposes(ops.rng_state(dev) if advance else None,
                                                table=(W, V, sel.op.rowptr, gn0, saved, None), zero=acc_all, head=head)
            st["emb_table"], st["emb_saved"] = sel, saved
            first_gn = (saved, ACT_NONE, p, 1)
        elif _PROLOGUE_DONE and not advance and acc_all is None and head is None:
            pass
        else:
            emb._glass_arena.refresh_transposes(ops.rng_state(dev) if advance else None, zero=acc_all, head=head)
        st["rng_epoch"] = ops.rng_epoch(dev)
        st["rng_words"] = ops.rng_snapshot(dev) if (snapshot_rng and advance and keep) else None
        ops._rng_cur[ops._dev(dev)] = st["rng_words"]
        if first_gn is not None:
            pass
        elif use_table:
            sel = emb._selection(x_flat)
            saved = torch.empty(4 * H, **f32)
            table = torch.empty((V, H), **f32)
            rng = ops.rng_tensor(dev).data_ptr() if p > 0 else 0
            _check(lib.glass_embed_norm_fwd_f32(x_flat.data_ptr(), W.data_ptr(), V, sel.op.rowptr.data_ptr(),
                                                gn0.weight.data_ptr(), gn0.bias.data_ptr(), gn0.mean_scale.data_ptr(),
                                                float(gn0.eps), saved.data_ptr(), table.data_ptr(),
                                                zp, pp, npos, p, rng, 1, h.data_ptr(), H,
                                                mask.data_ptr(), n, H, _stream()), "glass_embed_norm_fwd_f32")
            st["emb_table"], st["emb_saved"] = sel, saved
        else:
            h0 = torch.empty((n, H), **f32)
            _check(lib.glass_embed_label_f32(x_flat.data_ptr(), W.data_ptr(), V, zp, pp, npos, h0.data_ptr(), H,
                                             mask.data_ptr(), n, H, _stream()),
                   "glass_embed_label_f32")
            st["h0"] = h0
            st["emb_saved"] = _GN(gn0).fwd(h0, h, ACT_NONE, p, 1)
        C_out = H * L if emb.jk else H
        jk = torch.empty((n, C_out), **f32)
        layers, cstats = [], []
        pending_gn = None
        c_prev = None
        for l, conv in enumerate(emb.convs):
            if conv.adj is None:
                conv.adj = buildAdj(edge_index, edge_weight, n, conv.aggr)
            pc = float(conv.dropout) if train else 0.0
            T = torch.empty((n, 2 * H), **f32)
            m = torch.empty((n, H), **f32)
            if pending_gn is None and first_gn is not None:
                _dual_fwd(W, None, conv._stack["trans"], mask, conv.z_ratio, act, T, m, gn=(*first_gn, h), xa_index=x_flat)
            elif pending_gn is None:
                _dual_fwd(h, None, conv._stack["trans"], mask, conv.z_ratio, act, T, m)
            else:
                h = torch.empty((n, H), **f32)
                _dual_fwd(c_prev, None, conv._stack["trans"], mask, conv.z_ratio, act, T, m, gn=(*pending_gn, h))
            a = conv.adj.fwd.spmm(m)
            g = torch.empty((n, H), **f32)
            gsaved = _GN(conv.gn).stats(a) if acc_fwd is None else _GN(conv.gn).stats_exact(a, acc_fwd[l])
            last = l + 1 == L
            c = jk[:, l * H:(l + 1) * H] if emb.jk else (jk if last else torch.empty((n, H), **f32))
            if unl and last:
                cstat = None
                _comb_eff_fwd(a, h, conv, mask, c, None, (gsaved, ACT_NONE, pc, conv.call_base, g), labels)
            elif _comb_eff_fwd_ok(conv, labels, H, _comb_eff_ld(emb, H)):
                cstat = acc_fwd[L + l] if acc_fwd is not None else \
                    torch.empty((int(lib.glass_comb_eff_fwd_blocks(n, H, labels.cap)), 2, H), dtype=torch.float64, device=dev)
                _comb_eff_fwd(a, h, conv, mask, c, cstat, (gsaved, ACT_NONE, pc, conv.call_base, g), labels)
            else:
                cstat = acc_fwd[L + l] if acc_fwd is not None else \
                    torch.empty((-(-n // st["stat_rows"]), 2, H), dtype=torch.float64, device=dev)
                _dual_fwd(a, h, conv._stack["comb"], mask, conv.z_ratio, ACT_NONE, None, c, cstat,
                          gn=(gsaved, ACT_NONE, pc, conv.call_base, g))
            cstats.append(cstat)
            rec = {"h": h, "T": T, "a": a, "g": g, "gsaved": getattr(gsaved, "saved", gsaved), "c": c, "pc": pc}
            if not last:
                if acc_fwd is not None:
                    nsaved = _PendingStats(torch.empty(4 * H, **f32), cstat, 1, emb.gns[l], REP_DENSE)
                else:
                    nsaved = _GN(emb.gns[l]).finalize([cstat], n)
                rec["nsaved"] = getattr(nsaved, "saved", nsaved)
                pending_gn, c_prev = (nsaved, act, p, conv.call_base + 1), c
            layers.append(rec if keep else None)
        st["jk"], st["layers"] = jk, layers
        if unl:
            return jk, (st if keep else None)
        gnf = _GN(emb.gns[-1])
        if acc_fwd is not None:
            st["final_saved"] = _PendingStats(torch.empty(4 * C_out, **f32), acc_fwd[L:] if emb.jk else acc_fwd[2 * L - 1],
                                              L if emb.jk else 1, emb.gns[-1], REP_DENSE)
        else:
            st["final_saved"] = gnf.finalize(cstats if emb.jk else cstats[-1:], n)
# ... 62 lines not shown
        dh_next = None
        npart = None
        pending = []
        nblk = -(-n // st["stat_rows"])
        f64 = dict(dtype=torch.float64, device=dev)
        for l in range(L - 1, -1, -1):
            conv, rec = emb.convs[l], st["layers"][l]
            last = l + 1 == L
            dc_src = None
            if last:
                dc = djk[:, l * H:(l + 1) * H] if emb.jk else djk
            elif (USE_GN_BWD_IN_COMB and npart.dtype == torch.int64 and _comb_eff_ok(conv, st.get("labels"), H, _comb_eff_ld(emb, H)) and
                  _lib.load().glass_comb_eff_bwd_gn_src_supported(n, H)):
                m = emb.gns[l]
                ad = djk[:, l * H:(l + 1) * H] if emb.jk else None
                dc_src = _lib.GnBwdSrc(npart.data_ptr(), _rep(npart), dh_next.data_ptr(), dh_next.stride(0), rec["c"].data_ptr(),
                                       rec["c"].stride(0), 0 if ad is None else ad.data_ptr(), 0 if ad is None else ad.stride(0),
                                       rec["nsaved"].data_ptr(), m.weight.data_ptr(), m.mean_scale.data_ptr(),
                                       m.weight.grad.data_ptr(), m.bias.grad.data_ptr(), m.mean_scale.grad.data_ptr(), acc, act,
                                       float(p), conv.call_base + 1)
                dc = dh_next
            else:
                dc = torch.empty((n, H), **f32)
                _GN(emb.gns[l]).bwd_from_stats(dh_next, rec["c"], rec["nsaved"], dc, npart, act, p, conv.call_base + 1,
                                               addend=djk[:, l * H:(l + 1) * H] if emb.jk else None, acc=acc)
            din = torch.empty((n, 2 * H), **f32)
            labels = st.get("labels")
            acc_all = st.get("gn_exact")
            if acc_all is not None:
                gpart = acc_all[2 * l]
            if acc_all is not None and _comb_eff_ok(conv, labels, H, _comb_eff_ld(emb, H)):
                _comb_eff_bwd(dc, conv, mask, din, rec["g"], rec["h"], pending, acc,
                              (gpart, rec["a"], rec["gsaved"], conv.gn.mean_scale, ACT_NONE, rec["pc"], conv.call_base), labels,
                              dsrc_gn=dc_src)
            elif acc_all is not None:
                _dual_bwd(dc, None, conv._stack["comb"], mask, conv.z_ratio, ACT_NONE, 2 * H, None, din, rec["g"], rec["h"],
                          pending, acc, gn=(gpart, rec["a"], rec["gsaved"], conv.gn.mean_scale, ACT_NONE, rec["pc"], conv.call_base))
            elif _comb_eff_ok(conv, labels, H, _comb_eff_ld(emb, H)):
                gpart = torch.empty((int(_lib.load().glass_comb_eff_blocks(n, H, labels.cap)), 2, H), **f64)
                _comb_eff_bwd(dc, conv, mask, din, rec["g"], rec["h"], pending, acc,
                              (gpart, rec["a"], rec["gsaved"], conv.gn.mean_scale, ACT_NONE, rec["pc"], conv.call_base), labels)
            else:
                gpart = torch.empty((nblk, 2, H), **f64)
                _dual_bwd(dc, None, conv._stack["comb"], mask, conv.z_ratio, ACT_NONE, 2 * H, None, din, rec["g"], rec["h"],
                          pending, acc, gn=(gpart, rec["a"], rec["gsaved"], conv.gn.mean_scale, ACT_NONE, rec["pc"], conv.call_base))
            da = torch.empty((n, H), **f32)
            _GN(conv.gn).bwd_from_stats(din[:, :H], rec["a"], rec["gsaved"], da, gpart, ACT_NONE, rec["pc"], conv.call_base,
                                        acc=acc)
            dm = conv.adj.bwd.spmm(da)
            dh = torch.empty((n, H), **f32)
            drop = (p, 1) if (l == 0 and "emb_table" in st) else None
            gn = None
            if l > 0:
                below, cb = st["layers"][l - 1], emb.convs[l - 1]
                npart = acc_all[2 * l - 1] if acc_all is not None else torch.empty((nblk, 2, H), **f64)
                gn = (npart, below["c"], below["nsaved"], emb.gns[l - 1].mean_scale, act, p, cb.call_base + 1)
            _dual_bwd(dm, rec["T"], conv._stack["trans"], mask, conv.z_ratio, act, H, din[:, H:], dh, rec["h"], None, pending,
                      acc, drop, gn)
            dh_next = dh
            st["layers"][l] = None
        W = emb.input_emb.weight
        self.applied_optimizer = False
        if st.get("unlabeled"):
            _reduce_pending(pending, None)
            if tail_hook is not None:
                tail_hook()
            sel = st["emb_table"]
            if acc:
                W.grad.add_(sel.op.spmm(dh_next))
            else:
                sel.op.spmm(dh_next, out=W.grad)
            return
        gn0 = emb.emb_gn
        fused_tail = "emb_table" in st and USE_FUSED_TAIL
        prod = _reduce_pending(pending, (st["emb_table"], dh_next) if fused_tail else None)
        if tail_hook is not None:
            tail_hook()
        if fused_tail:
            sel, arena = st["emb_table"], emb._glass_arena
            offs = [arena.offset_of(t) for t in (W, gn0.weight, gn0.bias, gn0.mean_scale)]
            opt_ok = fused_opt is not None and all(o is not None for o in offs) and fused_opt.fusable() and acc == 0
            G, ws, rrows, n_red = prod
            oargs = (*fused_opt.fused_args(), *offs) if opt_ok else (0, 0, 0, 0, 0, 0, 0.0, 0.0, 0.0, 0.0, 0, 0, 0, 0, 0)
            _check(_lib.load().glass_embed_norm_bwd_adam_f32(G.data_ptr(), W.data_ptr(), W.shape[0], sel.op.rowptr.data_ptr(),
                                                             gn0.weight.data_ptr(), gn0.mean_scale.data_ptr(),
                                                             st["emb_saved"].data_ptr(), W.grad.data_ptr(), acc,
                                                             gn0.weight.grad.data_ptr(), gn0.bias.grad.data_ptr(),
                                                             gn0.mean_scale.grad.data_ptr(), acc, H, ws, rrows, n_red,
                                                             *oargs, _stream()),
                   "glass_embed_norm_bwd_adam_f32")
            self.applied_optimizer = opt_ok
            return
        if "emb_table" in st:
            sel = st["emb_table"]
            G = sel.op.spmm(dh_next)
            _check(_lib.load().glass_embed_norm_bwd_f32(G.data_ptr(), W.data_ptr(), W.shape[0], sel.op.rowptr.data_ptr(),
                                                        gn0.weight.data_ptr(), gn0.mean_scale.data_ptr(),
                                                        st["emb_saved"].data_ptr(), W.grad.data_ptr(), acc,
                                                        gn0.weight.grad.data_ptr(), gn0.bias.grad.data_ptr(),
                                                        gn0.mean_scale.grad.data_ptr(), acc, H, _stream()),
                   "glass_embed_norm_bwd_f32")
            return
        dh0 = torch.empty((n, H), **f32)
        _GN(gn0).bwd(dh_next, st["h0"], st["emb_saved"], dh0, ACT_NONE, p, 1, acc=acc)
        if acc:
            W.grad.add_(emb._selection(st["x_flat"]).op.spmm(dh0))
        else:
            emb._selection(st["x_flat"]).op.spmm(dh0, out=W.grad)


    def written_params(self, head):
        emb = self.emb
        if not hasattr(emb, "emb_gn"):
            out = [emb.input_emb.weight]
            for gn in [c.gn for c in emb.convs] + list(emb.gns):
                out += [gn.weight, gn.bias, gn.mean_scale]
            for c in emb.convs:
                out += [c.trans_fn.weight, c.trans_fn.bias, c.comb_fn.weight, c.comb_fn.bias]
            return out
        out = [emb.input_emb.weight, head.weight, head.bias]
        for gn in [emb.emb_gn] + [c.gn for c in emb.convs] + list(emb.gns):
            out += [gn.weight, gn.bias, gn.mean_scale]
        for c in emb.convs:
            for lin in list(c.trans_fns) + list(c.comb_fns):
                out += [lin.weight, lin.bias]
        return out

    def loss_and_grads(self, x_flat, z, edge_index, edge_weight, pos, pool_mode, head, target, loss_mode, overwrite=False,
                       tail_hook=None, labels=None, fused_opt=None):
        with torch.no_grad():
            (loss, logits), st = self.forward(x_flat, z, edge_index, edge_weight, True,
                                              readout=(pos, pool_mode, head, target, loss_mode), acc=0 if overwrite else 1,
                                              labels=labels)
            self.backward(st, None, tail_hook, fused_opt if overwrite else None)
        return loss, logits


_ones = {}


def _one(device):
    t = _ones.get(device)
    if t is None:
        t = _ones[device] = torch.ones((), dtype=torch.float32, device=device)
    return t


def step_supported(model, loss_fn):
    import torch.nn as nn
    from . import losses
    from .models import EmbZGConv, PoolModule
    emb = getattr(model, "conv", None)
    if not (USE_READOUT and isinstance(emb, EmbZGConv) and StackProgram.supported(emb) and emb.training):
        return False
    pool, head = model.pools[0], model.preds[0]
    if not (isinstance(pool, PoolModule) and pool.trans_fn is None and pool.mode in ("sum", "mean", "size")):
        return False
    if not (type(head) is nn.Linear and head.bias is not None and head.weight.grad is not None and
            head.bias.grad is not None and losses.fusable_mode(loss_fn) is not None):
        return False
    C = emb.gns[-1].weight.shape[0]
    return head.weight.shape[1] == C and bool(_lib.load().glass_readout_supported(C, head.weight.shape[0],
                                                                                  _lib.POOL_MODES[pool.mode]))


def covers_arena(model, arena):
    prog = _program(model.conv)
    return {id(p) for p in arena.params} <= {id(p) for p in prog.written_params(model.preds[0])}


def _program(emb):
    prog = emb.__dict__.get("_glass_stack_prog")
    if prog is None:
        prog = emb.__dict__["_glass_stack_prog"] = StackProgram(emb)
    return prog


def loss_and_grads(model, loss_fn, x, edge_index, edge_weight, pos, z, target, overwrite=False, tail_hook=None, labels=None,
                   fused_opt=None):
    """(loss, logits) of model(x, ..., pos, z) under loss_fn, gradients accumulated in place (see step_supported).
    z = "pos": label the nodes listed in pos (what utils.MaxZOZ(x, pos) would mark) without materialising z."""
    from . import losses
    emb = model.conv
    if x.dim() != 3 or x.shape[1] != 1 or x.shape[2] != 1:
        raise NotImplementedError("one integer feature per node (x of shape [N,1,1])")
    x_flat = x.reshape(x.shape[0])
    if x_flat.dtype != torch.int64:
        x_flat = x_flat.to(torch.int64)
    prog = _program(emb)
    pos = pos.contiguous()
    if pos.dtype != torch.int64:
        pos = pos.to(torch.int64)
    if isinstance(z, str):
        if z != "pos":
            raise ValueError("z must be a tensor, None or 'pos'")
        z = ("pos", pos)
    return prog.loss_and_grads(x_flat, z, edge_index, edge_weight, pos, model.pools[0].mode, model.preds[0], target,
                               losses.fusable_mode(loss_fn), overwrite, tail_hook, labels, fused_opt)


def applied_optimizer(model):
    return bool(getattr(_program(model.conv), "applied_optimizer", False))


class StackFn(torch.autograd.Function):
    @staticmethod
    def forward(ctx, prog, x_flat, z, edge_index, edge_weight, *params):
        keep = any(ctx.needs_input_grad)
        out, st = prog.forward(x_flat, z, edge_index, edge_weight, keep, snapshot_rng=True)
        ctx.prog, ctx.st, ctx.n_in = prog, st, 5 + len(params)
        return out

    @staticmethod
    def backward(ctx, dout):
        st, ctx.st = ctx.st, None
        if st is None:
            raise RuntimeError("StackFn: backward called twice (activations are released after the first pass)")
        dout, _ = ops._rows(dout)
        ctx.prog.backward(st, dout)
        return (None, ) * ctx.n_in


def run(emb, x_flat, z, edge_index, edge_weight):
    prog = _program(emb)
    params = [p for p in emb.parameters() if p.requires_grad]
    return StackFn.apply(prog, x_flat, z, edge_index, edge_weight, *params)
```

### glass_amd/step.py

```python
import os

import torch

from . import dist as gdist
from . import utils


CAPTURE_COLLECTIVE = os.environ.get("GLASS_CAPTURE_COLLECTIVE", "1") != "0"
VERIFY_CAPTURED_COLLECTIVE = os.environ.get("GLASS_VERIFY_CAPTURED_COLLECTIVE", "1") != "0"
_VERIFY_TOL = 1e-5


class TrainStep:
    def __init__(self, model, optimizer, loss_fn, x, edge_index, edge_weight, bucket=None, use_graph=True,
                 warmup_iters=3, preserve_state=False):
        self.model, self.opt, self.loss_fn = model, optimizer, loss_fn
        self.x, self.ei, self.ew = x, edge_index, edge_weight
        self.bucket = bucket if bucket is not None else gdist.bucket_for(model)
        self.use_graph = use_graph
        self.warmup_iters = warmup_iters
        self.preserve_state = preserve_state
        self.graphed = False
        self._pos = self._y = None
        self._labels = None
        self._loss = torch.zeros((), device=x.device)
        self._loss_sum = torch.zeros((), dtype=torch.float32, device=x.device)
        self._hyper = None
        self._one = torch.ones((), device=x.device)
        self._g_fb = self._g_tail = None
        self._split = False
        self._comm_stream = None
        self.time_collective = False
        self._coll_events = []
        self.collective_in_graph = False
        self.capture_error = None
        self.capture_verified = None
        self._force_verify_mismatch = False
        self._force_capture_failure = False
        self.exchange_enabled = True
        self._head_sig = None
        self._recapture = False

    def _fused_head(self):
        import torch.nn as nn
        from . import losses
        head = self.model.preds[0]
        return losses.fusable_mode(self.loss_fn) is not None and type(head) is nn.Linear and head.bias is not None

    def _program_step(self):
        from . import stack
        return (self._fused_head() and hasattr(self.bucket, "flat_param") and self.x.dim() == 3 and
                self.x.shape[1:] == (1, 1) and stack.step_supported(self.model, self.loss_fn))

    def _fwd_bwd(self, tail_hook=None, apply_opt=False):
        from . import stack
        if self._program_step():
            overwrite = stack.covers_arena(self.model, self.bucket)
            if not overwrite:
                self.bucket.zero()
            fused = self.opt if (apply_opt and overwrite and hasattr(self.opt, "fused_args")) else None
            prog = stack._program(self.model.conv)
            prog.loss_sum = self._loss_sum
            try:
                loss, _logits = stack.loss_and_grads(self.model, self.loss_fn, self.x, self.ei, self.ew, self._pos, "pos",
                                                     self._y, overwrite, tail_hook, labels=self._labels, fused_opt=fused)
            finally:
                prog.loss_sum = None
            self._loss = loss
            return stack.applied_optimizer(self.model)
        if tail_hook is not None:
            raise RuntimeError("tail_hook needs the step program")
        z = utils.MaxZOZ(self.x, self._pos)
        self.bucket.zero()
        if self._fused_head():
            from . import losses
            emb = self.model.NodeEmb(self.x, self.ei, self.ew, z)
            pooled = self.model.Pool(emb, self._pos, self.model.pools[0])
            loss, _logits = losses.head_loss(pooled, self.model.preds[0], self._y, losses.fusable_mode(self.loss_fn),
                                             direct=hasattr(self.bucket, "flat_param"))
        else:
            pred = self.model(self.x, self.ei, self.ew, self._pos, z, id=0)
            loss = self.loss_fn(pred, self._y)
        loss.backward(gradient=self._one)
        self._loss = loss.detach()
        self._loss_sum.add_(self._loss)

    def _warmup(self):
        snap = None
        if self.preserve_state and self.warmup_iters > 0:
            snap = self._snapshot()
        side = torch.cuda.Stream()
        side.wait_stream(torch.cuda.current_stream())
        with torch.cuda.stream(side):
            for _ in range(self.warmup_iters):
                solo = not gdist.is_distributed()
                done = self._fwd_bwd(apply_opt=solo)
                self.bucket.all_reduce_mean()
                if not done:
                    self.opt.step()
        torch.cuda.current_stream().wait_stream(side)
        torch.cuda.synchronize()
        if snap is not None:
            self._restore(snap)

    def _snapshot(self):
        import copy
        from . import ops
        return (copy.deepcopy(self.model.state_dict()), copy.deepcopy(self.opt.state_dict()),
                {k: getattr(self.opt, k).clone() for k in ("exp_avg", "exp_avg_sq", "step_dev", "step_dev_shard") if hasattr(self.opt, k)},
                ops.rng_state(self.x.device).clone(), self._loss_sum.clone())

    def _restore(self, snap):
        from . import ops
        self.model.load_state_dict(snap[0])
        self.opt.load_state_dict(snap[1])
        for k, v in snap[2].items():
            getattr(self.opt, k).copy_(v)
        ops.rng_state(self.x.device).copy_(snap[3])
        self._loss_sum.copy_(snap[4])
        torch.cuda.synchronize()

    def _verify_collective_capture(self):
        import torch.distributed as td
        snap = self._snapshot()
        head = self._labels is not None and self._labels.in_head
        if head:
            self._labels.rewind()
        self._fwd_bwd()
        self.bucket.all_reduce_mean()
        self.opt.step()
        torch.cuda.synchronize()
        g_eager, p_eager = self.bucket.flat.clone(), self.bucket.flat_param.clone()
        self._restore(snap)
        if head:
            self._labels.rewind()
        self._g_fb.replay()
        torch.cuda.synchronize()
        g_graph, p_graph = self.bucket.flat.clone(), self.bucket.flat_param.clone()
        self._restore(snap)

        def rel(a, b):
            d = float(b.abs().max())
            e = float((a - b).abs().max())
            return e / (d if d > 0 else 1.0) if (e == e and d == d) else float("inf")
        e_g, e_p = rel(g_graph, g_eager), rel(p_graph, p_eager)
        bad = 1.0 if (self._force_verify_mismatch or not (e_g <= _VERIFY_TOL and e_p <= _VERIFY_TOL)) else 0.0
        flag = torch.tensor([bad], device=self.x.device)
        td.all_reduce(flag, op=td.ReduceOp.MAX)
        ok = float(flag.item()) == 0.0
        self.capture_verified = {"grad_rel_inf": e_g, "param_rel_inf": e_p, "ok": ok, "tol": _VERIFY_TOL}
        return ok

    def _overlap_small_bucket(self):
        return (gdist.is_distributed() and hasattr(self.bucket, "sharded") and self.bucket.sharded() and
                self._program_step())

    def _capture(self):
        dist_on = gdist.is_distributed()
        self._g_fb = torch.cuda.CUDAGraph()
        mode = "thread_local" if dist_on else "global"
        if dist_on:
            torch.cuda.synchronize()
        if not dist_on:
            with torch.cuda.graph(self._g_fb):
                if not self._fwd_bwd(apply_opt=True):
                    self.opt.step()
        elif not self._overlap_small_bucket():
            import torch.distributed as td
            if CAPTURE_COLLECTIVE and td.get_backend() == "nccl":
                try:
                    if self._force_capture_failure:
                        raise RuntimeError("forced capture failure (test hook)")
                    g = torch.cuda.CUDAGraph()
                    with torch.cuda.graph(g, capture_error_mode=mode):
                        self._fwd_bwd()
                        self.bucket.all_reduce_mean()
                        self.opt.step()
                    self._g_fb, self.collective_in_graph = g, True
                except Exception as e:
                    self.capture_error = repr(e)
                    torch.cuda.synchronize()
                    self._g_fb = torch.cuda.CUDAGraph()
                ok = torch.tensor([1.0 if self.collective_in_graph else 0.0], device=self.x.device)
                td.all_reduce(ok, op=td.ReduceOp.MIN)
                if float(ok.item()) == 0.0 and self.collective_in_graph:
                    self.capture_error = "another rank could not capture the collective: split form on every rank"
                    self.collective_in_graph = False
                    self._g_fb = torch.cuda.CUDAGraph()
                if self.collective_in_graph and VERIFY_CAPTURED_COLLECTIVE and hasattr(self.bucket, "flat_param"):
                    if not self._verify_collective_capture():
                        self.capture_error = (f"captured collective failed the replay-vs-eager check: {self.capture_verified}")
                        self.collective_in_graph = False
                        self._g_fb = torch.cuda.CUDAGraph()
            if not self.collective_in_graph:
                with torch.cuda.graph(self._g_fb, capture_error_mode=mode):
                    self._fwd_bwd()
        else:
            self._g_tail = torch.cuda.CUDAGraph()
            self._comm_stream = torch.cuda.Stream()
            side = torch.cuda.Stream()
            side.wait_stream(torch.cuda.current_stream())
            with torch.cuda.stream(side):
                self._g_fb.capture_begin(capture_error_mode=mode)

                def cut():
                    self._g_fb.capture_end()
                    self._g_tail.capture_begin(pool=self._g_fb.pool(), capture_error_mode=mode)
                self._fwd_bwd(tail_hook=cut)
                self._g_tail.capture_end()
            torch.cuda.current_stream().wait_stream(side)
        self._split = dist_on and not self.collective_in_graph
        self.graphed = True

    def _exchange_and_update(self):
        ev = None
        if self.time_collective:
            ev = [torch.cuda.Event(enable_timing=True) for _ in range(3)]
            ev[0].record()
        if not self.exchange_enabled:
            if self._g_tail is not None:
                self._g_tail.replay()
        elif self._g_tail is not None:
            main, comm = torch.cuda.current_stream(), self._comm_stream
            ex = self.bucket.exchange
            comm.wait_stream(main)
            with torch.cuda.stream(comm):
                ex.reduce_small()
            self._g_tail.replay()
            ex.reduce_big()
            main.wait_stream(comm)
        else:
            self.bucket.all_reduce_mean()
        if ev:
            ev[1].record()
        self.opt.step()
        if ev:
            ev[2].record()
            self._coll_events = (self._coll_events + [ev])[-64:]

    def collective_share(self):
        import torch.distributed as td
        if not (td.is_available() and td.is_initialized()):
            return None
        backend = td.get_backend()
        out = {"world_size": td.get_world_size(), "backend": backend, "rccl_version": None,
               "in_graph": self.collective_in_graph, "collective_in_graph": self.collective_in_graph,
               "capture_error": self.capture_error, "capture_verified": self.capture_verified,
               "small_bucket_overlaps_backward_tail": self._g_tail is not None,
               "exchange_us": None, "adam_and_gather_us": None, "steps_timed": 0}
        if backend == "nccl":
            try:
                out["rccl_version"] = ".".join(str(v) for v in torch.cuda.nccl.version())
            except Exception as e:
                out["rccl_version"] = f"unavailable ({type(e).__name__})"
        ex = getattr(self.bucket, "exchange", None)
        if ex is not None:
            out["payload_bytes"] = ex.payload_bytes()
            out["world"] = ex.world
        else:
            out["payload_bytes"] = {"small_allreduce": self.bucket.flat.numel() * self.bucket.flat.element_size(),
                                    "big_reduce_scatter": 0, "big_all_gather": 0}
            out["world"] = td.get_world_size()
        out["predicted"] = gdist.predict_collective_us(out["payload_bytes"], out["world"])
        out["predicted_us"] = out["predicted"]["total_us"]
        if self._coll_events:
            torch.cuda.synchronize()
            red = [a.elapsed_time(b) * 1e3 for a, b, _ in self._coll_events]
            upd = [b.elapsed_time(c) * 1e3 for _, b, c in self._coll_events]
            out.update(exchange_us=sum(red) / len(red), adam_and_gather_us=sum(upd) / len(upd), steps_timed=len(red))
        return out

    def reset_loss_sum(self):
        self._loss_sum.zero_()

    def loss_sum(self):
        return self._loss_sum

    def _alloc_batch(self, shape, pos, y):
        self._pos = torch.full(shape, -1, dtype=pos.dtype, device=pos.device)
        self._y = torch.zeros((shape[0], ) + tuple(y.shape[1:]), dtype=y.dtype, device=y.device)
        if self._program_step() and pos.is_cuda and pos.dtype == torch.int64:
            from . import stack
            self._labels = stack.BatchLabels(self.x.shape[0], self._pos.numel(), pos.device)

    def begin_epoch(self, pos_all, y_all, idx_batches, wrap=False):
        if not (self.use_graph and pos_all.is_cuda and pos_all.dim() == 2 and pos_all.dtype == torch.int64 and
                pos_all.is_contiguous() and y_all.is_cuda and y_all.is_contiguous() and y_all.shape[0] == pos_all.shape[0] and
                idx_batches.is_cuda and idx_batches.dim() == 2 and idx_batches.dtype == torch.int64 and
                idx_batches.is_contiguous() and idx_batches.shape[0] > 0 and
                (y_all.element_size() * (y_all.numel() // max(y_all.shape[0], 1))) % 4 == 0):
            return False
        shape = (idx_batches.shape[1], ) + tuple(pos_all.shape[1:])
        first = self._pos is None
        if first:
            if not self._program_step():
                return False
            self._alloc_batch(shape, pos_all, y_all)
        if self._labels is None or shape != tuple(self._pos.shape) or y_all.dtype != self._y.dtype:
            return False
        was_head = self._labels.in_head
        self._labels.set_epoch(pos_all, y_all, idx_batches, self._pos, self._y, wrap=wrap)
        self._labels.in_head = True
        sig = self._labels.head_signature()
        hyper = self.opt.hyper() if hasattr(self.opt, "hyper") else None
        if first or not self.graphed or hyper != self._hyper or sig != self._head_sig or not was_head or self._recapture:
            if first:
                self._warmup()
            self._hyper, self._head_sig, self._recapture = hyper, sig, False
            self._capture()
            self._labels.set_epoch(pos_all, y_all, idx_batches, self._pos, self._y, wrap=wrap)
        return True

    def next_step(self):
        if hasattr(self.opt, "sync_lr"):
            self.opt.sync_lr()
        self._g_fb.replay()
        if self._split:
            self._exchange_and_update()
        return self._loss

    def __call__(self, pos, y, index=None):
        shape = tuple(pos.shape) if index is None else (index.numel(), ) + tuple(pos.shape[1:])
        first = self._pos is None
        if first:
            self._alloc_batch(shape, pos, y)
        if shape != tuple(self._pos.shape):
            raise ValueError("TrainStep needs a fixed batch shape (drop_last=True): "
                             f"{shape} vs {tuple(self._pos.shape)}")
        if self._labels is not None and self._labels.in_head:
            self._labels.in_head = False
            self._recapture = self.graphed
        self._load_batch(pos, y, index)
        hyper = self.opt.hyper() if hasattr(self.opt, "hyper") else None
        if first or (self.graphed and (hyper != self._hyper or self._recapture)):
            self._recapture = False
            if first:
                self._warmup()
            self._hyper = hyper
            if self.use_graph:
                self._capture()
        if hasattr(self.opt, "sync_lr"):
            self.opt.sync_lr()
        if self.graphed:
            self._g_fb.replay()
            if self._split:
                self._exchange_and_update()
        elif gdist.is_distributed():
            self._fwd_bwd()
            self._exchange_and_update()
        elif not self._fwd_bwd(apply_opt=True):
            self.opt.step()
        return self._loss

    def _load_batch(self, pos, y, index=None):
        if index is not None:
            index = index.contiguous()
            if (self._labels is not None and pos.is_contiguous() and y.is_cuda and y.is_contiguous() and index.is_cuda and
                    index.dtype == torch.int64 and index.is_contiguous() and y.dtype == self._y.dtype and pos.dim() == 2 and
                    y.shape[0] == pos.shape[0] and (y.element_size() * (y.numel() // max(y.shape[0], 1))) % 4 == 0):
                self._labels.load_gather(pos, y, index, self._pos, self._y)
                return
            pos, y = pos[index], y[index]
        if self._labels is not None:
            pos_c = pos if pos.is_contiguous() else pos.contiguous()
            if (y.is_cuda and y.is_contiguous() and y.dtype == self._y.dtype and y.shape == self._y.shape and y.numel() and
                    (y.element_size() * y.numel()) % 4 == 0):
                self._labels.load(pos_c, self._pos, y, self._y)
            else:
                self._labels.load(pos_c, self._pos)
                self._y.copy_(y)
            return
        if (pos.is_cuda and y.is_cuda and pos.is_contiguous() and y.is_contiguous() and pos.dtype == self._pos.dtype and
                y.dtype == self._y.dtype and y.shape == self._y.shape and pos.numel() and y.numel() and
                (pos.element_size() * pos.numel()) % 4 == 0 and (y.element_size() * y.numel()) % 4 == 0):
            from . import _lib
            rc = _lib.load().glass_copy_pair(self._pos.data_ptr(), pos.data_ptr(), pos.numel() * pos.element_size(),
                                             self._y.data_ptr(), y.data_ptr(), y.numel() * y.element_size(),
                                             torch.cuda.current_stream().cuda_stream)
            _lib.check(rc, "glass_copy_pair")
            return
        self._pos.copy_(pos)
        self._y.copy_(y)

    def last_loss(self):
        return float(self._loss.item())
```

### include/glass_hip.h

```cpp
#ifndef GLASS_HIP_H
#define GLASS_HIP_H

#include <stdint.h>

#ifdef __cplusplus
extern "C" {

typedef struct glass_gn_bwd_src glass_gn_bwd_src;
typedef struct glass_gn_src glass_gn_src;
#endif

#define GLASS_ABI_VERSION 6

#define GLASS_E_ARG (-1)
#define GLASS_E_PLAN (-2)
#define GLASS_E_UNSUPPORTED (-3)
#define GLASS_E_WS (-4)

#define GLASS_POOL_SUM 0
#define GLASS_POOL_MEAN 1
#define GLASS_POOL_MAX 2
#define GLASS_POOL_SIZE 3

#define GLASS_ACT_MASK 0xff
// ... 156 lines not shown
                                uint64_t gn_call_id, int gn_exact, void* stream);
int glass_dual_linear_bwd_f32(const float* dsrc, int64_t ldd, const float* T, int64_t ldt, const uint8_t* mask,
                              double z_ratio, int act, const float* WTimg, int64_t n_out, const float* addend,
                              int64_t ldadd, float p_drop, const uint64_t* rng_state, uint64_t call_id, float* out,
                              int64_t ldo, int64_t n_nodes, int64_t H, double* gn_partial, const float* gn_x,
                              int64_t gn_ldx, const float* gn_saved, const float* gn_alpha, int gn_act, float gn_p_drop,
                              uint64_t gn_call_id, int gn_exact, const float* X, int64_t ldx, const float* X2, int64_t ldx2,
                              void* ws, void* stream);
int glass_dual_linear_wgrad_f32(const float* dsrc, int64_t ldd, const float* T, int64_t ldt, const uint8_t* mask,
                                double z_ratio, int act, const float* X, int64_t ldx, const float* X2, int64_t ldx2,
                                int64_t N, int64_t H, float* dW, int64_t lddw, float* db, int accumulate, void* ws,
                                void* stream);
int glass_comb_eff_supported(int64_t H);
int glass_comb_eff_fwd_supported(int64_t H);
int glass_comb_eff_fwd_layout(int64_t H);
int glass_comb_eff_dgrad_layout2(int64_t H);
int64_t glass_comb_eff_max_rows(int64_t ld);
int64_t glass_comb_eff_blocks(int64_t n_nodes, int64_t H, int64_t lab_cap);
int64_t glass_comb_eff_fwd_blocks(int64_t n_nodes, int64_t H, int64_t lab_cap);
int64_t glass_comb_eff_ws_bytes(int64_t n_nodes, int64_t H, int64_t lab_cap);
int glass_comb_eff_fwd_f32(const float* xa, int64_t lda, const float* xb, int64_t ldb, const float* Wimg_eff,
                           const float* bias, const uint8_t* mask, double z_ratio, float* out, int64_t ldo,
                           int64_t n_nodes, int64_t H, double* stats, int stats_exact, const float* gn_saved,
                           const glass_gn_src* gn_src, int gn_act, float p_drop, const uint64_t* rng_state,
                           uint64_t call_id, float* xa_out, int64_t ldxo, const int32_t* lab_rows,
                           const int32_t* lab_count, int64_t lab_cap, void* stream);
struct glass_gn_bwd_src {
    const int64_t* acc;
    int64_t n_rep;
    const float* dy;
    int64_t lddy;
    const float* x;
    int64_t ldx;
    const float* addend;
    int64_t ldadd;
    const float *saved, *gamma, *alpha;
    float *dgamma, *dbeta, *dalpha;
    int accumulate, act;
    float p_drop;
    uint64_t call_id;
};
int glass_comb_eff_bwd_gn_src_supported(int64_t n_nodes, int64_t H);
int glass_comb_eff_bwd_f32(const float* dsrc, int64_t ldd, const uint8_t* mask, double z_ratio, const float* WTimg_eff,
                           float* out, int64_t ldo, int64_t n_nodes, int64_t H, double* gn_partial, const float* gn_x,
                           int64_t gn_ldx, const float* gn_saved, const float* gn_alpha, int gn_act, float gn_p_drop,
                           const uint64_t* rng_state, uint64_t gn_call_id, int gn_exact, const float* X, int64_t ldx,
                           const float* X2, int64_t ldx2, void* ws, const int32_t* lab_rows, const int32_t* lab_count,
                           int64_t lab_cap, const glass_gn_bwd_src* dsrc_gn, void* stream);
int glass_linear_wgrad_reduce_batch_f32(int64_t n_jobs, const void* const* ws, const int64_t* N, const int64_t* O,
                                        const int64_t* I, float* const* dW, const int64_t* lddw, float* const* db,
                                        const int32_t* accumulate, const int64_t* lab_cap, void* stream);
int glass_wgrad_reduce_spmm_f32(int64_t n_jobs, const void* const* ws, const int64_t* N, const int64_t* O, const int64_t* I,
                                float* const* dW, const int64_t* lddw, float* const* db, const int32_t* accumulate,
                                const int64_t* lab_cap, const int32_t* rowptr, const int32_t* col, const float* val,
                                const float* X, int64_t ldx, float* Y, int64_t ldy, int64_t n_rows, int64_t H,
                                const int32_t* plan_header_host, const int32_t* plan_dev, void* ws_spmm, void* stream);
int glass_spmm_reduce_rows_f32(const float* partials, float* Y, int64_t ldy, int64_t H, const int32_t* reduce_rows_dev,
                               int64_t n_reduce, void* stream);
int64_t glass_dense_image_floats(int64_t NT, int64_t KT, int32_t flags);
int glass_dense_pack_batch_f32(const float* const* src, float* const* dst, const int64_t* dst_floats, const int64_t* NT,
                               const int64_t* KT, const int32_t* flags, const float* z_ratio, int64_t n_jobs,
                               uint64_t* rng_state, void* stream);
int glass_step_prologue_f32(const float* const* src, float* const* dst, const int64_t* dst_floats, const int64_t* NT,
                            const int64_t* KT, const int32_t* flags, const float* z_ratio, int64_t n_jobs, uint64_t* rng_state,
                            const float* W, int64_t V, const int32_t* class_rowptr, const float* gamma, const float* beta,
                            const float* alpha, float eps, float* saved, float* table, int64_t H, int64_t* zero_words,
                            int64_t n_zero_words, void* stream);
typedef struct glass_batch_cursor {
    const int64_t* pos_all;
    const void* y_all;
    const int64_t* idx;
    int64_t n_all;
    int64_t n_batches;
    int64_t cursor;
    int64_t wrap;
} glass_batch_cursor;
int glass_step_head_f32(const float* const* src, float* const* dst, const int64_t* dst_floats, const int64_t* NT,
                        const int64_t* KT, const int32_t* flags, const float* z_ratio, int64_t n_jobs, uint64_t* rng_state,
                        const float* W, int64_t V, const int32_t* class_rowptr, const float* gamma, const float* beta,
                        const float* alpha, float eps, float* saved, float* table, int64_t H, int64_t* zero_words,
                        int64_t n_zero_words, glass_batch_cursor* cur, int64_t n_idx, int64_t smax, int64_t y_row_bytes,
                        int64_t* pos_dst, void* y_dst, uint8_t* mask, int32_t* lab_rows, int32_t* lab_count, void* ws,
                        int64_t n_nodes, void* stream);
typedef struct glass_peer_group {
    int32_t world, rank;
    const float* grad[8];
    uint64_t* flags[8];
} glass_peer_group;
int glass_peer_allreduce_adam_f32(const glass_peer_group* grp, int64_t n, float* param, float* exp_avg, float* exp_avg_sq,
                                  const float* lr_dev, double beta1, double beta2, double eps, double weight_decay,
                                  int64_t* step_dev, uint64_t* seq_dev, int32_t* status_dev, int64_t spin_limit,
                                  float* mean_out, void* stream);
int glass_peer_alloc(int64_t bytes, void** out);
int glass_peer_free(void* p);
int glass_peer_export(void* p, void* handle64);
int glass_peer_import(const void* handle64, void** out);
int glass_peer_close(void* p);
struct glass_gn_src {
    const int64_t* acc;
    int64_t n_src;
    int64_t n_rep;
    const float *gamma, *beta, *alpha;
    float eps;
};
int glass_gn_exact_supported(int64_t H);
int glass_gn_exact_fwd_supported(int64_t H);
int64_t glass_gn_exact_words(int64_t C);
int glass_graphnorm_stats_exact_f32(const float* x, int64_t ldx, int64_t n_rows, int64_t C, int64_t* acc, int n_rep,
                                    void* stream);

int glass_head_loss_fwd_f32(const float* pooled, int64_t ldp, const float* W, const float* bias, const void* target,
                            int mode, int64_t B, int64_t C, int64_t K, float* logits, float* prob, float* loss,
                            void* stream);
int glass_head_loss_bwd_f32(const float* pooled, int64_t ldp, const float* W, const float* prob, const void* target,
                            int mode, const float* grad_loss, int64_t B, int64_t C, int64_t K, float* dpooled,
                            int64_t lddp, float* dW, float* db, int accumulate, void* stream);

int glass_head_linear_f32(const float* pooled, int64_t ldp, const float* W, const float* bias, int64_t B, int64_t C, int64_t K,
                          float* logits, int64_t ldl, void* stream);

int glass_graphnorm_stats_f32(const float* x, int64_t ldx, int64_t n_rows, int64_t C, const float* gamma,
                              const float* beta, const float* alpha, float eps, float* saved, void* ws, void* stream);
int glass_readout_supported(int64_t C, int64_t K, int pool_mode);
int64_t glass_readout_ws_bytes(int64_t B, int64_t C, int64_t K);
int64_t glass_readout_scatter_ws_bytes(int64_t n_nodes, int64_t B, int64_t Smax);
int glass_readout_train_f32(const float* jk, int64_t ldj, const float* gn_saved, const float* gamma, const float* alpha,
                            const int64_t* pos, int64_t B, int64_t Smax, int pool_mode, const float* Wh, const float* bh,
                            const void* target, int loss_mode, int64_t K, const float* grad_loss, float* pooled,
                            float* logits, float* loss, float* djk, int64_t lddj, float* dWh, float* dbh, int acc_head,
                            float* dgamma, float* dbeta, float* dalpha, int acc_gn, void* ws, int64_t n_nodes, int64_t C,
                            const uint8_t* mask, const int32_t* lab_rows, const int32_t* lab_count,
                            const glass_gn_src* gn_src, int64_t* gn_bwd_acc, int gn_bwd_rep, void* scatter_ws,
                            float* loss_sum, void* stream);

int glass_copy_pair(void* dst0, const void* src0, int64_t bytes0, void* dst1, const void* src1, int64_t bytes1,
                    void* stream);

int glass_adam_step_f32(float* param, const float* grad, float* exp_avg, float* exp_avg_sq, int64_t n,
                        const float* lr_dev, double beta1, double beta2, double eps, double weight_decay,
                        int64_t* step_dev, void* stream);

#define GLASS_SEG_GCN 0
#define GLASS_SEG_GIN 1
#define GLASS_SEG_LDS_NODES 4096
int glass_seg_extract_count(const int32_t* in_rowptr, const int32_t* in_col, const float* in_w,
                            const int32_t* out_rowptr, const int32_t* out_col, int64_t n_base,
                            const int32_t* sub_ptr, const int32_t* sub_nodes, int64_t n_sub, int64_t n_member, int mode,
                            int32_t* cnt_in, int32_t* cnt_out, float* deg, void* stream);
int glass_seg_extract_fill(const int32_t* in_rowptr, const int32_t* in_col, const float* in_w,
                           const int32_t* out_rowptr, const int32_t* out_col, const float* out_w, int64_t n_base,
                           const int32_t* sub_ptr, const int32_t* sub_nodes, int64_t n_sub, int64_t n_member, int mode,
                           const float* deg, const int32_t* rowptr_in, const int32_t* rowptr_out,
                           int32_t* col_in, float* val_in, int32_t* col_out, float* val_out, void* stream);
int glass_seg_collate(const int32_t* sub_ptr, const int32_t* sub_nodes, int64_t n_sub,
                      const int32_t* rowptr_in, const int32_t* col_in, const float* val_in,
                      const int32_t* rowptr_out, const int32_t* col_out, const float* val_out,
                      const int32_t* ids, int64_t n_batch, const int32_t* node_off, int64_t n_nodes,
                      const int32_t* brow_in, const int32_t* brow_out,
                      int32_t* bcol_in, float* bval_in, int32_t* bcol_out, float* bval_out,
                      int32_t* node_map, int64_t* pos, int64_t pos_width, void* stream);

#define GLASS_SEG_KHOP_LDS_NODES 131072
#define GLASS_SEG_KHOP_WS_SLOTS 1024
int64_t glass_seg_khop_ws_bytes(int64_t n_base, int64_t n_sub);
int glass_seg_khop_count(const int32_t* in_rowptr, const int32_t* in_col, int64_t n_base, const int32_t* sub_ptr,
                         const int32_t* sub_nodes, int64_t n_sub, int64_t n_member, int hops, void* ws,
// ... 10 lines not shown
```

Before: 5.516 billion edges/s.

## Carry next step's head work into the last tail launch of the graphed step

Adds a step_tail kernel that fuses the embedding-norm backward and Adam with the next step's head work: weight repacking, embedding table rebuild, zeroing and label loading. The captured graph then runs headless, dropping the separate head launch at the start of each replay. A cold-entry path runs the head manually and rewinds rng and cursor state whenever the carried state is stale. This adds signature tracking and state-rollback logic that must stay consistent with the rng and cursor versions.

```diff
diff --git a/glass_amd/_lib.py b/glass_amd/_lib.py
--- a/glass_amd/_lib.py
+++ b/glass_amd/_lib.py
@@ -108,6 +108,10 @@
     "glass_peer_close": (c_int, [_P]),
     "glass_step_head_f32": (c_int, [_P, _P, _P, _P, _P, _P, _P, _I, _P, _P, _I, _P, _P, _P, _P, c_float, _P, _P, _I, _P, _I,
                                     _P, _I, _I, _I, _P, _P, _P, _P, _P, _P, _I, _P]),
+    "glass_step_tail_f32": (c_int, [_P, _P, _I, _P, _P, _P, _P, _P, c_int, _P, _P, _P, c_int, _I, _P, _P, _I, _P, _P, _P,
+                                    _P, _I, _P, c_double, c_double, c_double, c_double, _P, _I, _I, _I, _I,
+                                    _P, _P, _P, _P, _P, _P, _P, _I, _P, _P, c_float, _P, _P, _P, _I,
+                                    _P, _I, _I, _I, _P, _P, _P, _P, _P, _P, _I, _P]),
     "glass_graphnorm_finalize_f32": (c_int, [_P, _I, _I, _I, _I, _P, _P, _P, c_float, _P, _P]),
     "glass_graphnorm_apply_f32": (c_int, [_P, _I, _P, _I, _I, _I, _P, c_int, c_float, _P, c_uint64, _P]),
     "glass_dual_linear_dgrad_f32": (c_int, [_P, _I, _P, _I, _P, c_double, c_int, _P, _I, _P, _I, c_float, _P, c_uint64, _P, _I,
diff --git a/glass_amd/arena.py b/glass_amd/arena.py
--- a/glass_amd/arena.py
+++ b/glass_amd/arena.py
@@ -189,6 +189,7 @@
     def refresh_transposes(self, rng_state=None, table=None, zero=None, head=None):
         src, dst, cap, nt, kt, tr, zr, k = self._pack_args
         from . import _lib, ops
+        self.prologue_calls = getattr(self, "prologue_calls", 0) + 1
         for i, p in enumerate(self._packs):
             zr[i] = float(getattr(p[5], "z_ratio", 0.0))
         if k == 0 and rng_state is not None and table is None and zero is None and head is None:
@@ -225,6 +226,22 @@
             if rng_state is not None and i == 0:
                 ops.note_rng_advance(rng_state.device)
 
+    def carrying_tail(self, tail_args, rng_state, table, zero, head):
+        src, dst, cap, nt, kt, tr, zr, k = self._pack_args
+        from . import _lib
+        if k > 16 or table is None or head is None:
+            raise RuntimeError("carrying_tail: needs the embedding-table path, labels in the head launch and at most 16 weight images")
+        for i, p in enumerate(self._packs):
+            zr[i] = float(getattr(p[5], "z_ratio", 0.0))
+        W, V, rowptr, gn, saved, tab = table
+        zargs = (0, 0) if zero is None else (zero.data_ptr(), zero.numel())
+        rc = _lib.load().glass_step_tail_f32(*tail_args, src.ctypes.data, dst.ctypes.data, cap.ctypes.data, nt.ctypes.data,
+                                             kt.ctypes.data, tr.ctypes.data, zr.ctypes.data, k,
+                                             0 if rng_state is None else rng_state.data_ptr(), gn.bias.data_ptr(), float(gn.eps),
+                                             saved.data_ptr(), 0 if tab is None else tab.data_ptr(), *zargs, *head.head_args(),
+                                             torch.cuda.current_stream().cuda_stream)
+        _lib.check(rc, "glass_step_tail_f32")
+
     def offset_of(self, param):
         return self._offsets.get(id(param))
 
diff --git a/glass_amd/csrc/dense.hip b/glass_amd/csrc/dense.hip
--- a/glass_amd/csrc/dense.hip
+++ b/glass_amd/csrc/dense.hip
@@ -4,6 +4,7 @@
 #include "split_mma.h"
 #include "wgrad_common.h"
 #include "emb_table.h"
+#include "emb_tail.h"
 
 #ifndef GLASS_WGRAD_STAGED
 #define GLASS_WGRAD_STAGED 0
@@ -2700,6 +2701,99 @@
     int64_t n;
 };
 
+__device__ __forceinline__ void pack_job_body(const PackJob& j, int bx, int gx, int nthr, int slice = 0, int nslices = 1) {
+    const int total = j.NT * j.KT / 4;
+    const int half_rows = (j.transposed ? j.KT : j.NT) / 2;
+    auto skip = [&](int n, int k) {
+        return nslices > 1 && (((j.transposed ? k : n) % half_rows) >> 2) % nslices != slice;
+    };
+    if (j.layout == kLayoutWave16 || j.layout == kLayoutWave16Cols) {
+        const int KQ = j.KT / 4, NTILES = j.NT / 16;
+        const bool cols = j.layout == kLayoutWave16Cols;
+        for (int l = bx * nthr + (int)threadIdx.x; l < total; l += gx * nthr) {
+            const int lane = l & 63, v = (l >> 6) & 3, t = (l >> 8) % NTILES, kc = (l >> 8) / NTILES;
+            const int jj = lane & 15, q = lane >> 4;
+            const int n = cols ? 64 * (t >> 2) + 16 * (t & 3) + jj : tile_col(t, jj);
+            if (skip(n, q * KQ + kc * kKC + 4 * v)) continue;
+            reinterpret_cast<float4*>(j.dst)[l] = pack_fetch(j, n, q * KQ + kc * kKC + 4 * v);
+        }
+        return;
+    }
+    if (j.layout == kLayoutWave16EffFwd || j.layout == kLayoutWave16EffDgrad || j.layout == kLayoutWave16EffFwdCols ||
+        j.layout == kLayoutWave16EffDgradCols) {
+        const bool fwd = j.layout == kLayoutWave16EffFwd || j.layout == kLayoutWave16EffFwdCols;
+        const bool cols = j.layout == kLayoutWave16EffFwdCols || j.layout == kLayoutWave16EffDgradCols;
+        const int NTe = fwd ? j.NT / 2 : j.NT, KTe = fwd ? j.KT : j.KT / 2;
+        const int KQ = KTe / 4, NTILES = NTe / 16, per = NTe * KTe / 4;
+        const float zr = j.zr, omz = 1.f - j.zr;
+        for (int l = bx * nthr + (int)threadIdx.x; l < 2 * per; l += gx * nthr) {
+            const int img = l >= per, ll = img ? l - per : l;
+            const int lane = ll & 63, v = (ll >> 6) & 3, t = (ll >> 8) % NTILES, kc = (ll >> 8) / NTILES;
+            const int jj = lane & 15, q = lane >> 4;
+            const int n = cols ? 64 * (t >> 2) + 16 * (t & 3) + jj : tile_col(t, jj), k = q * KQ + kc * kKC + 4 * v;
+            if (skip(n, k)) continue;
+            const float4 a = pack_fetch(j, n, k);
+            const float4 b = fwd ? pack_fetch(j, j.NT / 2 + n, k) : pack_fetch(j, n, j.KT / 2 + k);
+            const float c1 = img ? zr : omz, c0 = img ? omz : zr;
+            reinterpret_cast<float4*>(j.dst)[l] = make_float4(c1 * a.x + c0 * b.x, c1 * a.y + c0 * b.y, c1 * a.z + c0 * b.z,
+                                                              c1 * a.w + c0 * b.w);
+        }
+        return;
+    }
+    if (j.layout == kLayoutTiledSplit) {
+        const int NKS = j.KT / 32;
+        for (int l = bx * nthr + (int)threadIdx.x; l < total; l += gx * nthr) {
+            const int nl = l & 255, q = (l >> 8) & 3, ks = l >> 10;
+            const int v = tiled_col(kLayoutTiledPlain, 0, nl, 0);
+            if (ks < NKS) {
+                const float4 e = pack_fetch(j, v % j.NT, (v / j.NT) * (j.KT / 2) + 16 * ks + 4 * q);
+                reinterpret_cast<float4*>(j.dst)[l] = e;
+                if (j.cut) pack_cut_put(j.dst + 4 * (size_t)total, ks, nl, q, e);
+            }
+        }
+        return;
+    }
+    const int NKS = j.KT / 16, H = j.NT / 2;
+    const int lay = j.layout == kLayoutTiledPlainEff ? kLayoutTiledPlain : j.layout == kLayoutTiledPairedEff ? kLayoutTiledPaired : j.layout;
+    const bool has_app = j.layout == kLayoutTiledPlainEff || j.layout == kLayoutTiledPairedEff;
+    float* cut = j.dst + 4 * (size_t)total + (has_app ? 2 * (size_t)total : 0);
+    for (int l = bx * nthr + (int)threadIdx.x; l < total; l += gx * nthr) {
+        const int nl = l & 255, q = (l >> 8) & 3, tile = l >> 10;
+        const int ct = tile / NKS, ks = tile % NKS;
+        const float4 e = pack_fetch(j, tiled_col(lay, ct, nl, H), 16 * ks + 4 * q);
+        reinterpret_cast<float4*>(j.dst)[l] = e;
+        if (j.cut) pack_cut_put(cut, tile, nl, q, e);
+    }
+    if (j.layout == kLayoutTiledPairedEff) {
+        float4* app = reinterpret_cast<float4*>(j.dst) + total;
+        const float zr = j.zr, omz = 1.f - j.zr;
+        for (int l = bx * nthr + (int)threadIdx.x; l < total / 2; l += gx * nthr) {
+            const int nl = l & 255, q = (l >> 8) & 3, tile = l >> 10;
+            const int ct = tile / NKS, ks = tile % NKS;
+            const int n = tiled_col(kLayoutTiledPlain, ct, nl, H), k = 16 * ks + 4 * q;
+            const float4 a = pack_fetch(j, n, k), b = pack_fetch(j, H + n, k);
+            const float4 e = make_float4(omz * a.x + zr * b.x, omz * a.y + zr * b.y, omz * a.z + zr * b.z, omz * a.w + zr * b.w);
+            app[l] = e;
+            if (j.cut) pack_cut_put(cut, total / 1024 + tile, nl, q, e);
+        }
+        return;
+    }
+    if (j.layout != kLayoutTiledPlainEff) return;
+    const int NKS2 = NKS / 2;
+    float4* app = reinterpret_cast<float4*>(j.dst) + total;
+    const float zr = j.zr, omz = 1.f - j.zr;
+    for (int l = bx * nthr + (int)threadIdx.x; l < total / 2; l += gx * nthr) {
+        const int nl = l & 255, q = (l >> 8) & 3, tile = l >> 10;
+        const int ct = tile / NKS2, ks = tile % NKS2;
+        const int n = tiled_col(kLayoutTiledPlain, ct, nl, H), k = 16 * ks + 4 * q;
+        const float4 a = pack_fetch(j, n, k), b = pack_fetch(j, n, j.KT / 2 + k);
+        const float4 e = make_float4(omz * a.x + zr * b.x, omz * a.y + zr * b.y, omz * a.z + zr * b.z, omz * a.w + zr * b.w);
+        app[l] = e;
+        if (j.cut) pack_cut_put(cut, total / 1024 + tile, nl, q, e);
+    }
+}
+
+
 __device__ __forceinline__ void pack_batch_body(const PackBatch& batch, uint64_t* rng_state, const TableJob& tab, int n_jobs,
                                                 const ZeroJob& zero, int rows) {
     if (rng_state && blockIdx.x == 0 && blockIdx.y == 0 && threadIdx.x == 0) rng_state[1] += 1;
@@ -2715,90 +2809,7 @@
                                 tab.table, tab_lds, tab_coef);
         return;
     }
-    const PackJob j = batch.job[blockIdx.y];
-    const int total = j.NT * j.KT / 4;
-    if (j.layout == kLayoutWave16 || j.layout == kLayoutWave16Cols) {
-        const int KQ = j.KT / 4, NTILES = j.NT / 16;
-        const bool cols = j.layout == kLayoutWave16Cols;
-        for (int l = blockIdx.x * kBlock + threadIdx.x; l < total; l += gridDim.x * kBlock) {
-            const int lane = l & 63, v = (l >> 6) & 3, t = (l >> 8) % NTILES, kc = (l >> 8) / NTILES;
-            const int jj = lane & 15, q = lane >> 4;
-            const int n = cols ? 64 * (t >> 2) + 16 * (t & 3) + jj : tile_col(t, jj);
-            reinterpret_cast<float4*>(j.dst)[l] = pack_fetch(j, n, q * KQ + kc * kKC + 4 * v);
-        }
-        return;
-    }
-    if (j.layout == kLayoutWave16EffFwd || j.layout == kLayoutWave16EffDgrad || j.layout == kLayoutWave16EffFwdCols ||
-        j.layout == kLayoutWave16EffDgradCols) {
-        const bool fwd = j.layout == kLayoutWave16EffFwd || j.layout == kLayoutWave16EffFwdCols;
-        const bool cols = j.layout == kLayoutWave16EffFwdCols || j.layout == kLayoutWave16EffDgradCols;
-        const int NTe = fwd ? j.NT / 2 : j.NT, KTe = fwd ? j.KT : j.KT / 2;
-        const int KQ = KTe / 4, NTILES = NTe / 16, per = NTe * KTe / 4;
-        const float zr = j.zr, omz = 1.f - j.zr;
-        for (int l = blockIdx.x * kBlock + threadIdx.x; l < 2 * per; l += gridDim.x * kBlock) {
-            const int img = l >= per, ll = img ? l - per : l;
-            const int lane = ll & 63, v = (ll >> 6) & 3, t = (ll >> 8) % NTILES, kc = (ll >> 8) / NTILES;
-            const int jj = lane & 15, q = lane >> 4;
-            const int n = cols ? 64 * (t >> 2) + 16 * (t & 3) + jj : tile_col(t, jj), k = q * KQ + kc * kKC + 4 * v;
-            const float4 a = pack_fetch(j, n, k);
-            const float4 b = fwd ? pack_fetch(j, j.NT / 2 + n, k) : pack_fetch(j, n, j.KT / 2 + k);
-            const float c1 = img ? zr : omz, c0 = img ? omz : zr;
-            reinterpret_cast<float4*>(j.dst)[l] = make_float4(c1 * a.x + c0 * b.x, c1 * a.y + c0 * b.y, c1 * a.z + c0 * b.z,
-                                                              c1 * a.w + c0 * b.w);
-        }
-        return;
-    }
-    if (j.layout == kLayoutTiledSplit) {
-        const int NKS = j.KT / 32;
-        for (int l = blockIdx.x * kBlock + threadIdx.x; l < total; l += gridDim.x * kBlock) {
-            const int nl = l & 255, q = (l >> 8) & 3, ks = l >> 10;
-            const int v = tiled_col(kLayoutTiledPlain, 0, nl, 0);
-            if (ks < NKS) {
-                const float4 e = pack_fetch(j, v % j.NT, (v / j.NT) * (j.KT / 2) + 16 * ks + 4 * q);
-                reinterpret_cast<float4*>(j.dst)[l] = e;
-                if (j.cut) pack_cut_put(j.dst + 4 * (size_t)total, ks, nl, q, e);
-            }
-        }
-        return;
-    }
-    const int NKS = j.KT / 16, H = j.NT / 2;
-    const int lay = j.layout == kLayoutTiledPlainEff ? kLayoutTiledPlain : j.layout == kLayoutTiledPairedEff ? kLayoutTiledPaired : j.layout;
-    const bool has_app = j.layout == kLayoutTiledPlainEff || j.layout == kLayoutTiledPairedEff;
-    float* cut = j.dst + 4 * (size_t)total + (has_app ? 2 * (size_t)total : 0);
-    for (int l = blockIdx.x * kBlock + threadIdx.x; l < total; l += gridDim.x * kBlock) {
-        const int nl = l & 255, q = (l >> 8) & 3, tile = l >> 10;
-        const int ct = tile / NKS, ks = tile % NKS;
-        const float4 e = pack_fetch(j, tiled_col(lay, ct, nl, H), 16 * ks + 4 * q);
-        reinterpret_cast<float4*>(j.dst)[l] = e;
-        if (j.cut) pack_cut_put(cut, tile, nl, q, e);
-    }
-    if (j.layout == kLayoutTiledPairedEff) {
-        float4* app = reinterpret_cast<float4*>(j.dst) + total;
-        const float zr = j.zr, omz = 1.f - j.zr;
-        for (int l = blockIdx.x * kBlock + threadIdx.x; l < total / 2; l += gridDim.x * kBlock) {
-            const int nl = l & 255, q = (l >> 8) & 3, tile = l >> 10;
-            const int ct = tile / NKS, ks = tile % NKS;
-            const int n = tiled_col(kLayoutTiledPlain, ct, nl, H), k = 16 * ks + 4 * q;
-            const float4 a = pack_fetch(j, n, k), b = pack_fetch(j, H + n, k);
-            const float4 e = make_float4(omz * a.x + zr * b.x, omz * a.y + zr * b.y, omz * a.z + zr * b.z, omz * a.w + zr * b.w);
-            app[l] = e;
-            if (j.cut) pack_cut_put(cut, total / 1024 + tile, nl, q, e);
-        }
-        return;
-    }
-    if (j.layout != kLayoutTiledPlainEff) return;
-    const int NKS2 = NKS / 2;
-    float4* app = reinterpret_cast<float4*>(j.dst) + total;
-    const float zr = j.zr, omz = 1.f - j.zr;
-    for (int l = blockIdx.x * kBlock + threadIdx.x; l < total / 2; l += gridDim.x * kBlock) {
-        const int nl = l & 255, q = (l >> 8) & 3, tile = l >> 10;
-        const int ct = tile / NKS2, ks = tile % NKS2;
-        const int n = tiled_col(kLayoutTiledPlain, ct, nl, H), k = 16 * ks + 4 * q;
-        const float4 a = pack_fetch(j, n, k), b = pack_fetch(j, n, j.KT / 2 + k);
-        const float4 e = make_float4(omz * a.x + zr * b.x, omz * a.y + zr * b.y, omz * a.z + zr * b.z, omz * a.w + zr * b.w);
-        app[l] = e;
-        if (j.cut) pack_cut_put(cut, total / 1024 + tile, nl, q, e);
-    }
+    pack_job_body(batch.job[blockIdx.y], blockIdx.x, gridDim.x, kBlock);
 }
 
 __global__ __launch_bounds__(kBlock) void pack_batch_kernel(PackBatch batch, uint64_t* rng_state, TableJob tab, int n_jobs,
@@ -2816,6 +2827,16 @@
     int64_t N;
 };
 
+__device__ __forceinline__ void label_job_body(const LabelJob& lj, int ahead) {
+    const int64_t n_b = lj.cur->n_batches, c = lj.cur->cursor, cb = c + ahead;
+    const int64_t b = cb < 0 ? 0 : (lj.cur->wrap ? cb % n_b : (cb >= n_b ? n_b - 1 : cb));
+    const BatchSrc src{lj.cur->pos_all, reinterpret_cast<const uint32_t*>(lj.cur->y_all), lj.cur->idx + b * lj.n_idx, lj.smax,
+                       lj.y_row_words > 0 ? lj.y_row_words : 1, lj.cur->n_all};
+    batch_labels_body<true>(src, lj.n_idx * lj.smax, lj.pos_dst, lj.y_dst, (int64_t)lj.n_idx * lj.y_row_words, lj.mask, lj.lab_rows,
+                            lj.lab_count, lj.owner, lj.N, 1);
+    if (threadIdx.x == 0) lj.cur->cursor = c + 1;
+}
+
 __global__ __launch_bounds__(kLabThreads) void step_head_kernel(PackBatch batch, uint64_t* rng_state, TableJob tab, int n_jobs,
                                                                 ZeroJob zero, int rows, LabelJob lj) {
     if ((int)blockIdx.y < rows) {
@@ -2824,13 +2845,72 @@
         return;
     }
     if (blockIdx.x != 0) return;
-    const int64_t n_b = lj.cur->n_batches, c = lj.cur->cursor;
-    const int64_t b = c < 0 ? 0 : (lj.cur->wrap ? c % n_b : (c >= n_b ? n_b - 1 : c));
-    const BatchSrc src{lj.cur->pos_all, reinterpret_cast<const uint32_t*>(lj.cur->y_all), lj.cur->idx + b * lj.n_idx, lj.smax,
-                       lj.y_row_words > 0 ? lj.y_row_words : 1, lj.cur->n_all};
-    batch_labels_body<true>(src, lj.n_idx * lj.smax, lj.pos_dst, lj.y_dst, (int64_t)lj.n_idx * lj.y_row_words, lj.mask, lj.lab_rows,
-                            lj.lab_count, lj.owner, lj.N, 1);
-    if (threadIdx.x == 0) lj.cur->cursor = c + 1;
+    label_job_body(lj, 0);
+}
+
+struct TailTable {
+    float* G;
+    const float* W;
+    int V, H;
+    const int32_t* rowptr;
+    const float *gamma, *alpha, *saved;
+    float* dW;
+    int accumulate_w;
+    float *dgamma, *dbeta, *dalpha;
+    int accumulate;
+    const float* partials;
+    const int32_t* rrows;
+    int n_reduce;
+};
+struct TailPack {
+    TailCover cover;
+    uint32_t jobs[kMaxTailCover];
+    int rows[kMaxTailCover], K[kMaxTailCover];
+    int nslices;
+};
+
+__global__ __launch_bounds__(kLabThreads) void step_tail_kernel(TailTable tt, TailAdam ad, int n_tab, PackBatch batch, TailPack tp,
+                                                                uint64_t* rng_state, TableJob tab, ZeroJob zero, LabelJob lj,
+                                                                int n_lin) {
+    __shared__ double lds[kBlock * 2];
+    __shared__ float coef[3 * kTabCols];
+    const int b = blockIdx.x, n_src = tp.cover.n * tp.nslices;
+    const bool wide = b >= n_tab && b <= n_tab + n_src;
+    if (!wide && threadIdx.x >= kBlock) return;
+    const int64_t step_now = ad.step[0] + 1;
+    const AdamCoef ac = adam_coef(step_now, ad.lr[0], ad.beta1, ad.beta2, ad.eps, ad.weight_decay);
+    if (b < n_tab) {
+        emb_tail_table_block(b, tt.G, tt.W, tt.V, tt.H, tt.rowptr, tt.gamma, tt.alpha, tt.saved, tt.dW, tt.accumulate_w, tt.dgamma,
+                             tt.dbeta, tt.dalpha, tt.accumulate, tt.partials, tt.rrows, tt.n_reduce, ad, ac, lds, coef);
+        __syncthreads();
+        emb_table_fwd_block(b, tab.W, tab.V, tab.H, tab.rowptr, tab.gamma, tab.beta, tab.alpha, tab.eps, tab.saved, tab.table, lds,
+                            coef);
+    } else if (b < n_tab + n_src) {
+        const int s = (b - n_tab) / tp.nslices, slice = (b - n_tab) % tp.nslices, S = tp.nslices;
+        const int K = tp.K[s], half = tp.rows[s] / 2, groups = half / 4;
+        const int mine = (groups - slice + S - 1) / S;
+        for (int e = threadIdx.x; e < mine * 8 * K; e += kLabThreads) {
+            const int gi = e / (8 * K), rem = e - gi * 8 * K, hf = rem / (4 * K), off = rem - hf * 4 * K;
+            const int64_t k = tp.cover.lo[s] + (int64_t)(hf * half + 4 * (slice + gi * S)) * K + off;
+            adam_update(ac, ad.p, ad.g[k], ad.m, ad.v, k);
+        }
+        __syncthreads();
+        const uint32_t feeds = tp.jobs[s];
+        for (int jb = 0; jb < kMaxPackJobs; ++jb) {
+            if (!((feeds >> jb) & 1u)) continue;
+            const PackJob j = batch.job[jb];
+            pack_job_body(j, 0, 1, kLabThreads, slice, S);
+        }
+    } else if (b == n_tab + n_src) {
+        if (rng_state && threadIdx.x == 0) rng_state[1] += 1;
+        label_job_body(lj, 1);
+    } else {
+        const int64_t wg = b - n_tab - n_src - 1;
+        if (zero.p)
+            for (int64_t k = wg * kBlock + threadIdx.x; k < zero.n; k += (int64_t)n_lin * kBlock) zero.p[k] = 0;
+        emb_tail_linear(ad, ac, tt.V, tt.H, wg, n_lin, &tp.cover);
+    }
+    adam_ticket(ad.step, step_now);
 }
 
 }
@@ -3493,13 +3573,10 @@
     return (g.part_w_floats + g.part_b_floats) * (int64_t)sizeof(float);
 }
 
-static int pack_launch(const float* const* src, float* const* dst, const int64_t* dst_floats, const int64_t* NT, const int64_t* KT,
-                       const int32_t* transposed, const float* z_ratio, int64_t n_jobs, uint64_t* rng_state,
-                       const TableJob& tab, void* stream, const char* what, ZeroJob zero = ZeroJob{nullptr, 0},
-                       const LabelJob* lj = nullptr) {
+static int pack_build(PackBatch& b, const float* const* src, float* const* dst, const int64_t* dst_floats, const int64_t* NT,
+                      const int64_t* KT, const int32_t* transposed, const float* z_ratio, int64_t n_jobs, const char* what) {
     GLASS_REQUIRE(n_jobs >= 0 && n_jobs <= kMaxPackJobs && (n_jobs == 0 || (src && dst && dst_floats && NT && KT && transposed)),
                   "%s: bad arguments (at most %d matrices per call)", what, kMaxPackJobs);
-    PackBatch b;
     for (int k = 0; k < kMaxPackJobs; ++k) b.job[k] = PackJob{nullptr, nullptr, 0, 0, 0, 0, 0.f, 0};
     for (int k = 0; k < n_jobs; ++k) {
         GLASS_REQUIRE(src[k] && dst[k] && NT[k] > 0 && NT[k] % 64 == 0 && KT[k] > 0 && KT[k] % 64 == 0 && aligned16(src[k]) &&
@@ -3529,6 +3606,15 @@
         b.job[k] = PackJob{src[k], dst[k], (int)NT[k], (int)KT[k], transposed[k] & 1, layout, z_ratio ? z_ratio[k] : 0.f,
                            tiled_layout ? 1 : 0};
     }
+    return 0;
+}
+
+static int pack_launch(const float* const* src, float* const* dst, const int64_t* dst_floats, const int64_t* NT, const int64_t* KT,
+                       const int32_t* transposed, const float* z_ratio, int64_t n_jobs, uint64_t* rng_state,
+                       const TableJob& tab, void* stream, const char* what, ZeroJob zero = ZeroJob{nullptr, 0},
+                       const LabelJob* lj = nullptr) {
+    PackBatch b;
+    if (const int rc = pack_build(b, src, dst, dst_floats, NT, KT, transposed, z_ratio, n_jobs, what)) return rc;
     unsigned gx = 32;
     if (tab.W && (unsigned)ceil_div(tab.H, kTabCols) > gx) gx = (unsigned)ceil_div(tab.H, kTabCols);
     unsigned gy = (unsigned)n_jobs + (tab.W ? 1u : 0u);
@@ -3598,3 +3684,82 @@
     return pack_launch(src, dst, dst_floats, NT, KT, transposed, z_ratio, n_jobs, rng_state, tab, stream, "glass_step_head_f32",
                        ZeroJob{n_zero_words > 0 ? (long long*)zero_words : nullptr, n_zero_words}, &lj);
 }
+
+extern "C" int glass_step_tail_f32(float* G, const float* W, int64_t V, const int32_t* class_rowptr, const float* gamma,
+                                   const float* alpha, const float* saved, float* dW, int accumulate_w, float* dgamma,
+                                   float* dbeta, float* dalpha, int accumulate, int64_t H, const float* partials,
+                                   const int32_t* reduce_rows, int64_t n_reduce, float* param, float* grad, float* exp_avg,
+                                   float* exp_avg_sq, int64_t n_param, const float* lr_dev, double beta1, double beta2,
+                                   double eps, double weight_decay, int64_t* step_dev, int64_t off_W, int64_t off_gamma,
+                                   int64_t off_beta, int64_t off_alpha, const float* const* src, float* const* dst,
+                                   const int64_t* dst_floats, const int64_t* NT, const int64_t* KT, const int32_t* transposed,
+                                   const float* z_ratio, int64_t n_jobs, uint64_t* rng_state, const float* beta, float gn_eps,
+                                   float* saved_next, float* table, int64_t* zero_words, int64_t n_zero_words,
+                                   glass_batch_cursor* cur, int64_t n_idx, int64_t smax, int64_t y_row_bytes, int64_t* pos_dst,
+                                   void* y_dst, uint8_t* mask, int32_t* lab_rows, int32_t* lab_count, void* ws, int64_t n_nodes,
+                                   void* stream) {
+    GLASS_REQUIRE(G && W && class_rowptr && gamma && alpha && beta && saved && saved_next && dW && dgamma && dbeta && dalpha,
+                  "step_tail: null pointer");
+    GLASS_REQUIRE(H > 0 && V > 0 && V <= GLASS_EMBED_NORM_MAX_ROWS && n_reduce >= 0 && (n_reduce == 0 || (partials && reduce_rows)),
+                  "step_tail: bad sizes");
+    GLASS_REQUIRE(param && grad && exp_avg && exp_avg_sq && lr_dev && step_dev && n_param > 0 && off_W >= 0 &&
+                      off_W + V * H <= n_param && off_gamma >= 0 && off_gamma + H <= n_param && off_beta >= 0 &&
+                      off_beta + H <= n_param && off_alpha >= 0 && off_alpha + H <= n_param && dW == grad + off_W &&
+                      W == param + off_W && dgamma == grad + off_gamma && dbeta == grad + off_beta &&
+                      dalpha == grad + off_alpha && gamma == param + off_gamma && beta == param + off_beta &&
+                      alpha == param + off_alpha,
+                  "step_tail: the table and emb_gn's vectors must be views of the arena at the given offsets");
+    GLASS_REQUIRE(n_zero_words >= 0 && (n_zero_words == 0 || zero_words), "step_tail: bad zero-fill arguments");
+    GLASS_REQUIRE(cur && pos_dst && mask && lab_rows && lab_count && ws, "step_tail: null pointer");
+    GLASS_REQUIRE(smax > 0 && n_idx > 0 && n_idx * smax < (1ll << 30) && n_nodes > 0 && n_nodes < (1ll << 31) &&
+                      (reinterpret_cast<uintptr_t>(cur) & 7u) == 0,
+                  "step_tail: bad sizes");
+    GLASS_REQUIRE(y_row_bytes == 0 || (y_dst && y_row_bytes > 0 && y_row_bytes % 4 == 0 && y_row_bytes < (1ll << 30) &&
+                                       (reinterpret_cast<uintptr_t>(y_dst) & 3u) == 0),
+                  "step_tail: the target rows have 4-byte granularity");
+    PackBatch b;
+    if (const int rc = pack_build(b, src, dst, dst_floats, NT, KT, transposed, z_ratio, n_jobs, "glass_step_tail_f32")) return rc;
+    TailPack tp{};
+    for (int k = 0; k < n_jobs; ++k) {
+        const int64_t lo = b.job[k].src - param, n = (int64_t)b.job[k].NT * b.job[k].KT;
+        GLASS_REQUIRE(b.job[k].src >= param && lo + n <= n_param, "step_tail: job %d reads a matrix outside the arena", k);
+        int s = 0;
+        while (s < tp.cover.n && tp.cover.lo[s] != lo) ++s;
+        if (s == tp.cover.n) {
+            tp.cover.lo[s] = lo;
+            tp.cover.hi[s] = lo + n;
+            tp.cover.n = s + 1;
+        }
+        GLASS_REQUIRE(tp.cover.hi[s] == lo + n, "step_tail: job %d reads the matrix at arena offset %lld with another size", k, (long long)lo);
+        tp.jobs[s] |= 1u << k;
+        tp.rows[s] = b.job[k].transposed ? b.job[k].KT : b.job[k].NT;
+        tp.K[s] = b.job[k].transposed ? b.job[k].NT : b.job[k].KT;
+        const int lay = b.job[k].layout;
+        GLASS_REQUIRE(lay == kLayoutWave16 || lay == kLayoutWave16Cols || lay == kLayoutWave16EffFwd || lay == kLayoutWave16EffDgrad ||
+                          lay == kLayoutWave16EffFwdCols || lay == kLayoutWave16EffDgradCols,
+                      "step_tail: job %d: only the wave16 layouts (hidden 64) are packed slice by slice", k);
+        GLASS_REQUIRE(tp.rows[s] % 8 == 0, "step_tail: job %d: the source is not a stacked pair of row groups", k);
+    }
+    tp.nslices = 16;
+    const int64_t own_lo[4] = {off_W, off_gamma, off_beta, off_alpha}, own_hi[4] = {off_W + V * H, off_gamma + H, off_beta + H, off_alpha + H};
+    for (int s = 0; s < tp.cover.n; ++s) {
+        for (int t = 0; t < s; ++t)
+            GLASS_REQUIRE(tp.cover.hi[t] <= tp.cover.lo[s] || tp.cover.hi[s] <= tp.cover.lo[t], "step_tail: packed matrices overlap in the arena");
+        for (int t = 0; t < 4; ++t)
+            GLASS_REQUIRE(own_hi[t] <= tp.cover.lo[s] || tp.cover.hi[s] <= own_lo[t], "step_tail: a packed matrix overlaps the embedding table or emb_gn");
+    }
+    const TailAdam ad{param, grad, exp_avg, exp_avg_sq, n_param, lr_dev, (float)beta1, (float)beta2, (float)eps,
+                      (float)weight_decay, step_dev, off_W, off_gamma, off_beta, off_alpha};
+    const TailTable tt{G, W, (int)V, (int)H, class_rowptr, gamma, alpha, saved, dW, accumulate_w, dgamma, dbeta, dalpha, accumulate,
+                       partials, reduce_rows, (int)n_reduce};
+    const TableJob tab{W, (int)V, (int)H, class_rowptr, gamma, beta, alpha, gn_eps, saved_next, table};
+    const LabelJob lj{cur, (int)n_idx, (int)smax, (int)(y_row_bytes / 4), pos_dst, (uint32_t*)y_dst, mask, lab_rows, lab_count,
+                      (int32_t*)ws, n_nodes};
+    const int n_tab = (int)ceil_div(H, kTabCols);
+    int64_t n_lin = ceil_div(std::max(n_param, n_zero_words), (int64_t)kBlock);
+    if (n_lin > 2048) n_lin = 2048;
+    hipLaunchKernelGGL(step_tail_kernel, dim3((unsigned)(n_tab + tp.cover.n * tp.nslices + 1 + n_lin)), dim3(kLabThreads), 0, (hipStream_t)stream, tt,
+                       ad, n_tab, b, tp, rng_state, tab, ZeroJob{n_zero_words > 0 ? (long long*)zero_words : nullptr, n_zero_words}, lj,
+                       (int)n_lin);
+    return launch_status("glass_step_tail_f32");
+}
diff --git a/glass_amd/csrc/emb_tail.h b/glass_amd/csrc/emb_tail.h
--- /dev/null
+++ b/glass_amd/csrc/emb_tail.h
@@ -0,0 +1,151 @@
+#pragma once
+#include "common.h"
+#include "emb_table.h"
+#include "gn_math.h"
+
+namespace glass {
+
+struct TailAdam {
+    float* p;
+    float* g;
+    float *m, *v;
+    int64_t n;
+    const float* lr;
+    float beta1, beta2, eps, weight_decay;
+    int64_t* step;
+    int64_t off_W, off_gamma, off_beta, off_alpha;
+};
+
+
+constexpr int kMaxTailCover = 16;
+struct TailCover {
+    int n;
+    int64_t lo[kMaxTailCover], hi[kMaxTailCover];
+};
+
+__device__ __forceinline__ void emb_tail_linear(const TailAdam& ad, const AdamCoef& ac, int V, int H, int64_t wg, int64_t n_wg,
+                                                const TailCover* cover) {
+    const int64_t tab_lo = ad.off_W, tab_hi = ad.off_W + (int64_t)V * H;
+    for (int64_t k = wg * kBlock + threadIdx.x; k < ad.n; k += n_wg * kBlock) {
+        if ((k >= tab_lo && k < tab_hi) || (k >= ad.off_gamma && k < ad.off_gamma + H) ||
+            (k >= ad.off_beta && k < ad.off_beta + H) || (k >= ad.off_alpha && k < ad.off_alpha + H))
+            continue;
+        if (cover) {
+            bool covered = false;
+            for (int s = 0; s < cover->n; ++s) covered = covered || (k >= cover->lo[s] && k < cover->hi[s]);
+            if (covered) continue;
+        }
+        adam_update(ac, ad.p, ad.g[k], ad.m, ad.v, k);
+    }
+}
+
+__device__ __forceinline__ void emb_tail_table_block(int blk, float* __restrict__ G, const float* W, int V, int H,
+                                                     const int32_t* __restrict__ rowptr, const float* gamma,
+                                                     const float* alpha, const float* saved, float* dW, int accumulate_w,
+                                                     float* dgamma, float* dbeta, float* dalpha, int accumulate,
+                                                     const float* __restrict__ partials, const int32_t* __restrict__ rrows,
+                                                     int n_reduce, const TailAdam& ad, const AdamCoef& ac, double* lds,
+                                                     float* coef) {
+    const int tc = threadIdx.x & (kTabCols - 1), tr = threadIdx.x / kTabCols;
+    const int c = blk * kTabCols + tc;
+    const bool ok = c < H;
+    constexpr int kOwn = 4;
+    const bool small = V <= kOwn * kTabSlots;
+    float w_own[kOwn], cn_own[kOwn], m_own[kOwn], v_own[kOwn];
+    if (small) {
+#pragma unroll
+        for (int k = 0; k < kOwn; ++k) {
+            const int v = tr + kTabSlots * k;
+            const bool live = ok && v < V;
+            const int64_t o = (int64_t)(live ? v : 0) * H + (ok ? c : 0);
+            w_own[k] = live ? W[o] : 0.f;
+            cn_own[k] = live ? (float)(rowptr[v + 1] - rowptr[v]) : 0.f;
+            m_own[k] = (live && ad.p) ? ad.m[ad.off_W + o] : 0.f;
+            v_own[k] = (live && ad.p) ? ad.v[ad.off_W + o] : 0.f;
+        }
+    }
+    if (ok)
+        for (int rr = tr; rr < n_reduce; rr += kTabSlots) {
+            const int row = rrows[3 * rr], first = rrows[3 * rr + 1], n = rrows[3 * rr + 2];
+            float sum = 0.f;
+            for (int k = 0; k < n; ++k) sum += partials[(int64_t)(first + k) * H + c];
+            G[(int64_t)row * H + c] = sum;
+        }
+    if (n_reduce > 0) __syncthreads();
+    double s1 = 0.0, s2 = 0.0;
+    float g_own[kOwn];
+    if (ok && small) {
+        const float mu = saved[c], rstd = saved[H + c], al = alpha[c];
+#pragma unroll
+        for (int k = 0; k < kOwn; ++k) {
+            const int v = tr + kTabSlots * k;
+            g_own[k] = v < V ? G[(int64_t)v * H + c] : 0.f;
+        }
+#pragma unroll
+        for (int k = 0; k < kOwn; ++k) {
+            if (tr + kTabSlots * k >= V) continue;
+            const float xhat = (w_own[k] - al * mu) * rstd;
+            s1 += (double)g_own[k];
+            s2 += (double)g_own[k] * (double)xhat;
+        }
+    } else if (ok) {
+        const float mu = saved[c], rstd = saved[H + c], al = alpha[c];
+        for (int v = tr; v < V; v += kTabSlots) {
+            const float g = G[(int64_t)v * H + c];
+            const float xhat = (W[(int64_t)v * H + c] - al * mu) * rstd;
+            s1 += (double)g;
+            s2 += (double)g * (double)xhat;
+        }
+    }
+    slot_reduce(s1, s2, lds, tc, tr);
+    if (tr == 0 && ok) {
+        float A, Bx, K, da;
+        gn_bwd_coeffs(s1, s2, (double)rowptr[V], gamma[c], alpha[c], saved[c], saved[H + c], A, Bx, K, da);
+        const float g_gamma = (accumulate ? dgamma[c] : 0.f) + (float)s2;
+        const float g_beta = (accumulate ? dbeta[c] : 0.f) + (float)s1;
+        const float g_alpha = (accumulate ? dalpha[c] : 0.f) + da;
+        dgamma[c] = g_gamma;
+        dbeta[c] = g_beta;
+        dalpha[c] = g_alpha;
+        coef[tc] = A;
+        coef[kTabCols + tc] = Bx;
+        coef[2 * kTabCols + tc] = K;
+        if (ad.p) {
+            adam_update(ac, ad.p, g_gamma, ad.m, ad.v, ad.off_gamma + c);
+            adam_update(ac, ad.p, g_beta, ad.m, ad.v, ad.off_beta + c);
+            adam_update(ac, ad.p, g_alpha, ad.m, ad.v, ad.off_alpha + c);
+        }
+    }
+    __syncthreads();
+    if (ok && small) {
+        const float A = coef[tc], Bx = coef[kTabCols + tc], K = coef[2 * kTabCols + tc];
+#pragma unroll
+        for (int k = 0; k < kOwn; ++k) {
+            const int v = tr + kTabSlots * k;
+            if (v >= V) continue;
+            const int64_t o = (int64_t)v * H + c;
+            float d = fmaf(A, g_own[k], cn_own[k] * fmaf(Bx, w_own[k], K));
+            if (accumulate_w) d += dW[o];
+            dW[o] = d;
+            if (ad.p) {
+                float pk = w_own[k];
+                adam_element(ac, pk, d, m_own[k], v_own[k]);
+                ad.m[ad.off_W + o] = m_own[k];
+                ad.v[ad.off_W + o] = v_own[k];
+                ad.p[ad.off_W + o] = pk;
+            }
+        }
+    } else if (ok) {
+        const float A = coef[tc], Bx = coef[kTabCols + tc], K = coef[2 * kTabCols + tc];
+        for (int v = tr; v < V; v += kTabSlots) {
+            const int64_t o = (int64_t)v * H + c;
+            const float cn = (float)(rowptr[v + 1] - rowptr[v]);
+            float d = fmaf(A, G[o], cn * fmaf(Bx, W[o], K));
+            if (accumulate_w) d += dW[o];
+            dW[o] = d;
+            if (ad.p) adam_update(ac, ad.p, d, ad.m, ad.v, ad.off_W + o);
+        }
+    }
+}
+
+}
diff --git a/glass_amd/csrc/embnorm.hip b/glass_amd/csrc/embnorm.hip
--- a/glass_amd/csrc/embnorm.hip
+++ b/glass_amd/csrc/embnorm.hip
@@ -1,5 +1,6 @@
 #include "common.h"
 #include "emb_table.h"
+#include "emb_tail.h"
 #include "gn_math.h"
 
 namespace glass {
@@ -66,17 +67,6 @@
     }
 }
 
-struct TailAdam {
-    float* p;
-    float* g;
-    float *m, *v;
-    int64_t n;
-    const float* lr;
-    float beta1, beta2, eps, weight_decay;
-    int64_t* step;
-    int64_t off_W, off_gamma, off_beta, off_alpha;
-};
-
 __global__ __launch_bounds__(kBlock) void emb_tail_kernel(float* __restrict__ G, const float* W, int V, int H,
                                                           const int32_t* __restrict__ rowptr,
                                                           const float* gamma, const float* alpha,
@@ -95,117 +85,12 @@
         ac = adam_coef(step_now, ad.lr[0], ad.beta1, ad.beta2, ad.eps, ad.weight_decay);
     }
     if ((int)blockIdx.x >= n_tab) {
-        const int64_t nb = (int64_t)gridDim.x - n_tab;
-        const int64_t tab_lo = ad.off_W, tab_hi = ad.off_W + (int64_t)V * H;
-        for (int64_t k = ((int64_t)blockIdx.x - n_tab) * kBlock + threadIdx.x; k < ad.n; k += nb * kBlock) {
-            if ((k >= tab_lo && k < tab_hi) || (k >= ad.off_gamma && k < ad.off_gamma + H) ||
-                (k >= ad.off_beta && k < ad.off_beta + H) || (k >= ad.off_alpha && k < ad.off_alpha + H))
-                continue;
-            adam_update(ac, ad.p, ad.g[k], ad.m, ad.v, k);
-        }
+        emb_tail_linear(ad, ac, V, H, (int64_t)blockIdx.x - n_tab, (int64_t)gridDim.x - n_tab, nullptr);
         adam_ticket(ad.step, step_now);
         return;
     }
-    const int tc = threadIdx.x & (kTabCols - 1), tr = threadIdx.x / kTabCols;
-    const int c = blockIdx.x * kTabCols + tc;
-    const bool ok = c < H;
-    constexpr int kOwn = 4;
-    const bool small = V <= kOwn * kTabSlots;
-    float w_own[kOwn], cn_own[kOwn], m_own[kOwn], v_own[kOwn];
-    if (small) {
-#pragma unroll
-        for (int k = 0; k < kOwn; ++k) {
-            const int v = tr + kTabSlots * k;
-            const bool live = ok && v < V;
-            const int64_t o = (int64_t)(live ? v : 0) * H + (ok ? c : 0);
-            w_own[k] = live ? W[o] : 0.f;
-            cn_own[k] = live ? (float)(rowptr[v + 1] - rowptr[v]) : 0.f;
-            m_own[k] = (live && ad.p) ? ad.m[ad.off_W + o] : 0.f;
-            v_own[k] = (live && ad.p) ? ad.v[ad.off_W + o] : 0.f;
-        }
-    }
-    if (ok)
-        for (int rr = tr; rr < n_reduce; rr += kTabSlots) {
-            const int row = rrows[3 * rr], first = rrows[3 * rr + 1], n = rrows[3 * rr + 2];
-            float sum = 0.f;
-            for (int k = 0; k < n; ++k) sum += partials[(int64_t)(first + k) * H + c];
-            G[(int64_t)row * H + c] = sum;
-        }
-    if (n_reduce > 0) __syncthreads();
-    double s1 = 0.0, s2 = 0.0;
-    float g_own[kOwn];
-    if (ok && small) {
-        const float mu = saved[c], rstd = saved[H + c], al = alpha[c];
-#pragma unroll
-        for (int k = 0; k < kOwn; ++k) {
-            const int v = tr + kTabSlots * k;
-            g_own[k] = v < V ? G[(int64_t)v * H + c] : 0.f;
-        }
-#pragma unroll
-        for (int k = 0; k < kOwn; ++k) {
-            if (tr + kTabSlots * k >= V) continue;
-            const float xhat = (w_own[k] - al * mu) * rstd;
-            s1 += (double)g_own[k];
-            s2 += (double)g_own[k] * (double)xhat;
-        }
-    } else if (ok) {
-        const float mu = saved[c], rstd = saved[H + c], al = alpha[c];
-        for (int v = tr; v < V; v += kTabSlots) {
-            const float g = G[(int64_t)v * H + c];
-            const float xhat = (W[(int64_t)v * H + c] - al * mu) * rstd;
-            s1 += (double)g;
-            s2 += (double)g * (double)xhat;
-        }
-    }
-    slot_reduce(s1, s2, lds, tc, tr);
-    if (tr == 0 && ok) {
-        float A, Bx, K, da;
-        gn_bwd_coeffs(s1, s2, (double)rowptr[V], gamma[c], alpha[c], saved[c], saved[H + c], A, Bx, K, da);
-        const float g_gamma = (accumulate ? dgamma[c] : 0.f) + (float)s2;
-        const float g_beta = (accumulate ? dbeta[c] : 0.f) + (float)s1;
-        const float g_alpha = (accumulate ? dalpha[c] : 0.f) + da;
-        dgamma[c] = g_gamma;
-        dbeta[c] = g_beta;
-        dalpha[c] = g_alpha;
-        coef[tc] = A;
-        coef[kTabCols + tc] = Bx;
-        coef[2 * kTabCols + tc] = K;
-        if (ad.p) {
-            adam_update(ac, ad.p, g_gamma, ad.m, ad.v, ad.off_gamma + c);
-            adam_update(ac, ad.p, g_beta, ad.m, ad.v, ad.off_beta + c);
-            adam_update(ac, ad.p, g_alpha, ad.m, ad.v, ad.off_alpha + c);
-        }
-    }
-    __syncthreads();
-    if (ok && small) {
-        const float A = coef[tc], Bx = coef[kTabCols + tc], K = coef[2 * kTabCols + tc];
-#pragma unroll
-        for (int k = 0; k < kOwn; ++k) {
-            const int v = tr + kTabSlots * k;
-            if (v >= V) continue;
-            const int64_t o = (int64_t)v * H + c;
-            float d = fmaf(A, g_own[k], cn_own[k] * fmaf(Bx, w_own[k], K));
-            if (accumulate_w) d += dW[o];
-            dW[o] = d;
-            if (ad.p) {
-                float pk = w_own[k];
-                adam_element(ac, pk, d, m_own[k], v_own[k]);
-                ad.m[ad.off_W + o] = m_own[k];
-                ad.v[ad.off_W + o] = v_own[k];
-                ad.p[ad.off_W + o] = pk;
-            }
-        }
-    } else if (ok) {
-        const float A = coef[tc], Bx = coef[kTabCols + tc], K = coef[2 * kTabCols + tc];
-        for (int v = tr; v < V; v += kTabSlots) {
-            const int64_t o = (int64_t)v * H + c;
-            const float cn = (float)(rowptr[v + 1] - rowptr[v]);
-            float d = fmaf(A, G[o], cn * fmaf(Bx, W[o], K));
-            if (accumulate_w) d += dW[o];
-            dW[o] = d;
-            if (ad.p) adam_update(ac, ad.p, d, ad.m, ad.v, ad.off_W + o);
-        }
-    }
+    emb_tail_table_block(blockIdx.x, G, W, V, H, rowptr, gamma, alpha, saved, dW, accumulate_w, dgamma, dbeta, dalpha,
+                         accumulate, partials, rrows, n_reduce, ad, ac, lds, coef);
     if (ad.p) adam_ticket(ad.step, step_now);
 }
 
diff --git a/glass_amd/stack.py b/glass_amd/stack.py
--- a/glass_amd/stack.py
+++ b/glass_amd/stack.py
@@ -24,6 +24,7 @@
 USE_FUSED_TAIL = os.environ.get("GLASS_FUSED_TAIL", "1") != "0"
 USE_GATHER_IN_TRANS = os.environ.get("GLASS_GATHER_IN_TRANS", "1") != "0"
 USE_COMB_EFF = os.environ.get("GLASS_COMB_EFF", "1") != "0"
+USE_CARRY_TAIL = os.environ.get("GLASS_CARRY_TAIL", "0") != "0"
 
 
 _PROLOGUE_DONE = False
@@ -501,8 +502,12 @@
         elif use_table and labels is not None and USE_GATHER_IN_TRANS and lib.glass_dual_linear_fwd_gather_supported(H):
             sel = emb._selection(x_flat)
             saved = torch.empty(4 * H, **f32)
-            emb._glass_arena.refresh_transposes(ops.rng_state(dev) if advance else None,
-                                                table=(W, V, sel.op.rowptr, gn0, saved, None), zero=acc_all, head=head)
+            pro = dict(rng_state=ops.rng_state(dev) if advance else None, table=(W, V, sel.op.rowptr, gn0, saved, None),
+                       zero=acc_all, head=head)
+            if head is not None and getattr(head, "carry", False):
+                st["carry"] = pro
+            else:
+                emb._glass_arena.refresh_transposes(**pro)
             st["emb_table"], st["emb_saved"] = sel, saved
             first_gn = (saved, ACT_NONE, p, 1)
         elif _PROLOGUE_DONE and not advance and acc_all is None and head is None:
@@ -731,13 +736,18 @@
             opt_ok = fused_opt is not None and all(o is not None for o in offs) and fused_opt.fusable() and acc == 0
             G, ws, rrows, n_red = prod
             oargs = (*fused_opt.fused_args(), *offs) if opt_ok else (0, 0, 0, 0, 0, 0, 0.0, 0.0, 0.0, 0.0, 0, 0, 0, 0, 0)
-            _check(_lib.load().glass_embed_norm_bwd_adam_f32(G.data_ptr(), W.data_ptr(), W.shape[0], sel.op.rowptr.data_ptr(),
-                                                             gn0.weight.data_ptr(), gn0.mean_scale.data_ptr(),
-                                                             st["emb_saved"].data_ptr(), W.grad.data_ptr(), acc,
-                                                             gn0.weight.grad.data_ptr(), gn0.bias.grad.data_ptr(),
-                                                             gn0.mean_scale.grad.data_ptr(), acc, H, ws, rrows, n_red,
-                                                             *oargs, _stream()),
-                   "glass_embed_norm_bwd_adam_f32")
+            targs = (G.data_ptr(), W.data_ptr(), W.shape[0], sel.op.rowptr.data_ptr(), gn0.weight.data_ptr(),
+                     gn0.mean_scale.data_ptr(), st["emb_saved"].data_ptr(), W.grad.data_ptr(), acc, gn0.weight.grad.data_ptr(),
+                     gn0.bias.grad.data_ptr(), gn0.mean_scale.grad.data_ptr(), acc, H, ws, rrows, n_red, *oargs)
+            self.carried = None
+            if st.get("carry") is not None:
+                if not (opt_ok and tail_hook is None):
+                    raise RuntimeError("headless step: the last launch cannot carry the next step's head work "
+                                       "(needs the fused optimizer step of one unsharded arena)")
+                arena.carrying_tail(targs, **st["carry"])
+                self.carried = st["carry"]
+            else:
+                _check(_lib.load().glass_embed_norm_bwd_adam_f32(*targs, _stream()), "glass_embed_norm_bwd_adam_f32")
             self.applied_optimizer = opt_ok
             return
         if "emb_table" in st:
@@ -811,6 +821,18 @@
     C = emb.gns[-1].weight.shape[0]
     return head.weight.shape[1] == C and bool(_lib.load().glass_readout_supported(C, head.weight.shape[0],
                                                                                   _lib.POOL_MODES[pool.mode]))
+
+
+def carry_supported(model, arena, opt):
+    emb = getattr(model, "conv", None)
+    if not (USE_CARRY_TAIL and USE_FUSED_TAIL and USE_EMBED_TABLE and USE_GATHER_IN_TRANS and hasattr(emb, "emb_gn") and
+            hasattr(opt, "fused_args") and opt.fusable() and getattr(emb, "_glass_arena", None) is arena):
+        return False
+    W, gn0 = emb.input_emb.weight, emb.emb_gn
+    V, H = W.shape
+    return (H == 64 and V <= _lib.EMBED_NORM_MAX_ROWS and bool(_lib.load().glass_dual_linear_fwd_gather_supported(H)) and
+            0 < arena._pack_args[7] <= 16 and covers_arena(model, arena) and
+            all(arena.offset_of(t) is not None for t in (W, gn0.weight, gn0.bias, gn0.mean_scale)))
 
 
 def covers_arena(model, arena):
diff --git a/glass_amd/step.py b/glass_amd/step.py
--- a/glass_amd/step.py
+++ b/glass_amd/step.py
@@ -40,6 +40,11 @@
         self.exchange_enabled = True
         self._head_sig = None
         self._recapture = False
+        self._headless = False
+        self._carry = None
+        self._carried = False
+        self._carry_sig = None
+        self.cold_entries = 0
 
     def _fused_head(self):
         import torch.nn as nn
@@ -155,16 +160,54 @@
         return (gdist.is_distributed() and hasattr(self.bucket, "sharded") and self.bucket.sharded() and
                 self._program_step())
 
+    def _carry_eligible(self):
+        from . import stack
+        return bool(self._labels is not None and self._labels.in_head and self._program_step() and
+                    hasattr(self.bucket, "flat_param") and stack.carry_supported(self.model, self.bucket, self.opt))
+
+    def _carry_signature(self):
+        from . import ops
+        return (getattr(self.bucket, "prologue_calls", 0), ops.rng_state(self.x.device)._version, self._labels.cursor._version,
+                self.bucket.flat_param._version, sum(p._version for p in self.bucket.params))
+
+    def _uncarry(self):
+        if self._carried:
+            from . import ops
+            rng = ops.rng_state(self.x.device)
+            if self._carry_sig is not None and rng._version == self._carry_sig[1]:
+                rng[1:2].sub_(1)
+            self._carried = False
+            self._carry_sig = None
+
+    def _cold_entry(self):
+        self._uncarry()
+        self.bucket.refresh_transposes(**self._carry)
+        self._labels.cursor[5:6].sub_(1)
+        self.cold_entries += 1
+
     def _capture(self):
+        self._uncarry()
+        self._headless, self._carry = False, None
         dist_on = gdist.is_distributed()
         self._g_fb = torch.cuda.CUDAGraph()
         mode = "thread_local" if dist_on else "global"
         if dist_on:
             torch.cuda.synchronize()
         if not dist_on:
-            with torch.cuda.graph(self._g_fb):
-                if not self._fwd_bwd(apply_opt=True):
-                    self.opt.step()
+            carry = self._carry_eligible()
+            self._labels_carry(carry)
+            try:
+                with torch.cuda.graph(self._g_fb):
+                    if not self._fwd_bwd(apply_opt=True):
+                        self.opt.step()
+            finally:
+                self._labels_carry(False)
+            if carry:
+                from . import stack
+                self._carry = stack._program(self.model.conv).carried
+                if self._carry is None:
+                    raise RuntimeError("headless capture: the step's last launch did not carry the head work")
+                self._headless = True
         elif not self._overlap_small_bucket():
             import torch.distributed as td
             if CAPTURE_COLLECTIVE and td.get_backend() == "nccl":
@@ -212,6 +255,10 @@
         self._split = dist_on and not self.collective_in_graph
         self.graphed = True
 
+    def _labels_carry(self, on):
+        if self._labels is not None:
+            self._labels.carry = bool(on)
+
     def _exchange_and_update(self):
         ev = None
         if self.time_collective:
@@ -314,6 +361,14 @@
     def next_step(self):
         if hasattr(self.opt, "sync_lr"):
             self.opt.sync_lr()
+        if self._headless:
+            cold = not self._carried or self._carry_signature() != self._carry_sig
+            if cold:
+                self._cold_entry()
+            self._g_fb.replay()
+            if cold:
+                self._carried, self._carry_sig = True, self._carry_signature()
+            return self._loss
         self._g_fb.replay()
         if self._split:
             self._exchange_and_update()
@@ -321,6 +376,7 @@
 
     def __call__(self, pos, y, index=None):
         shape = tuple(pos.shape) if index is None else (index.numel(), ) + tuple(pos.shape[1:])
+        self._uncarry()
         first = self._pos is None
         if first:
             self._alloc_batch(shape, pos, y)
diff --git a/include/glass_hip.h b/include/glass_hip.h
--- a/include/glass_hip.h
+++ b/include/glass_hip.h
@@ -262,6 +262,18 @@
                         int64_t n_zero_words, glass_batch_cursor* cur, int64_t n_idx, int64_t smax, int64_t y_row_bytes,
                         int64_t* pos_dst, void* y_dst, uint8_t* mask, int32_t* lab_rows, int32_t* lab_count, void* ws,
                         int64_t n_nodes, void* stream);
+int glass_step_tail_f32(float* G, const float* W, int64_t V, const int32_t* class_rowptr, const float* gamma,
+                        const float* alpha, const float* saved, float* dW, int accumulate_w, float* dgamma, float* dbeta,
+                        float* dalpha, int accumulate, int64_t H, const float* partials, const int32_t* reduce_rows,
+                        int64_t n_reduce, float* param, float* grad, float* exp_avg, float* exp_avg_sq, int64_t n_param,
+                        const float* lr_dev, double beta1, double beta2, double eps, double weight_decay, int64_t* step_dev,
+                        int64_t off_W, int64_t off_gamma, int64_t off_beta, int64_t off_alpha, const float* const* src,
+                        float* const* dst, const int64_t* dst_floats, const int64_t* NT, const int64_t* KT,
+                        const int32_t* flags, const float* z_ratio, int64_t n_jobs, uint64_t* rng_state, const float* beta,
+                        float gn_eps, float* saved_next, float* table, int64_t* zero_words, int64_t n_zero_words,
+                        glass_batch_cursor* cur, int64_t n_idx, int64_t smax, int64_t y_row_bytes, int64_t* pos_dst,
+                        void* y_dst, uint8_t* mask, int32_t* lab_rows, int32_t* lab_count, void* ws, int64_t n_nodes,
+                        void* stream);
 typedef struct glass_peer_group {
     int32_t world, rank;
     const float* grad[8];
```

Measured after the change: 5.541 billion edges/s (median of 6 runs). Within noise of the previous version (+0.5%).
